# ChainBreak/denoising_diffusion_deep_fake

Measured on AMD Instinct MI355X. Metric: training images/sec (256x256 U-Net, bs=16/GPU), higher is better.
Workload: dtype f32; 1 GPU; d3f train_denoiser step: noise blend -> Unet(resnet34) fwd -> (MSE+1-SSIM)/2 -> bwd -> Adam, 256x256 synthetic face crops, bs=16/GPU, random-init weights, train-mode BatchNorm; image_size=256, batch_per_gpu=16, global_batch=16, parallelism=dp1, graph_step=False, adam_overlap_tail=False, adam_overlap_tail_steps=0, ranks_seen=1, csrc_digest=87bcf01c09701563

## Files before the change

### denoising_diffusion_deep_fake_amd/_lib.py

```python
import ctypes as C
import os
import re
from pathlib import Path

_HERE = Path(__file__).resolve().parent
LIB_PATH = Path(os.environ["D3F_LIB"]) if os.environ.get("D3F_LIB") else _HERE / "csrc" / "libd3f_hip.so"
HEADER_PATH = _HERE.parent / "include" / "d3f_hip.h"

F32, BF16, F32X3 = 0, 1, 2
AUGMENT_NONE = -1


ACT_IDENTITY, ACT_SIGMOID, ACT_TANH, ACT_SOFTMAX, ACT_LOGSOFTMAX, ACT_CLAMP = range(6)
HEAD_ACTIVATIONS = {None: ACT_IDENTITY, "sigmoid": ACT_SIGMOID, "tanh": ACT_TANH, "softmax2d": ACT_SOFTMAX,
                    "logsoftmax": ACT_LOGSOFTMAX, "clamp": ACT_CLAMP}


RESAMPLE_CUBIC, RESAMPLE_CUBIC_AA = 0, 1
COLOR_NONE, COLOR_MEANSTD = 0, 1
COLOR_MATCH_MODES = {None: COLOR_NONE, "none": COLOR_NONE, "meanstd": COLOR_MEANSTD}


def color_match_mode(color_match):
    if not (color_match is None or isinstance(color_match, str)) or color_match not in COLOR_MATCH_MODES:
# ... 129 lines not shown
    "d3f_paste_resize_cubic_u8": (_i, [_p, _i, _i, _i, _i64, _p, _i, _i, _i, _i, _i, _i, _i, _p, _p]),
    "d3f_channel_sums_u8": (_i, [_p, _i, _i, _i, _i64, _p, _p]),
    "d3f_color_match_coef": (_i, [_p, _p, _i, _i64, _p, _p]),
    "d3f_paste_resize_cubic_color_u8": (_i, [_p, _i, _i, _i, _i64, _p, _i, _i, _i, _i, _i, _i, _i, _p, _p, _p]),
    "d3f_temporal_filter_u8": (_i, [_p, _i64, _p, _i64, _i, _i, _i, _p, _p, _p, _f, _i, _p]),
    "d3f_color_coef_smooth": (_i, [_p, _p, _i, _i64, _f, _p, _p, _p, _p]),
    "d3f_temporal_flag_set": (_i, [_p, _i, _p]),
    "d3f_unet_predict_frames_full_u8": (_i, [_p, _p, _p, _p, _i, _i, _i, _i, _i, _i, _i, _p, _p, C.POINTER(_f), C.POINTER(_f),
                                             _p, _i, _p]),
    "d3f_crop_resize_cubic_boxes_u8": (_i, [_p, _i, _i, _i, C.POINTER(C.c_int32), _p, _i, _i, _i64, _p]),
    "d3f_crop_resize_cubic_aa_boxes_u8": (_i, [_p, _i, _i, _i, C.POINTER(C.c_int32), _p, _i, _i, _i64, _p]),
    "d3f_paste_resize_cubic_boxes_u8": (_i, [_p, _i, _i, _i, _i64, _p, _i, _i, C.POINTER(C.c_int32), _i, _p, _p]),
    "d3f_paste_resize_cubic_color_boxes_u8": (_i, [_p, _i, _i, _i, _i64, _p, _i, _i, C.POINTER(C.c_int32), _i, _p, _p, _p]),
    "d3f_unet_predict_frames_boxes_u8": (_i, [_p, _p, _p, _p, _i, _i, C.POINTER(C.c_int32), _p, C.POINTER(_f), C.POINTER(_f),
                                              _p, _i, _p]),
    "d3f_unet_predict_frames_full_boxes_u8": (_i, [_p, _p, _p, _p, _i, _i, C.POINTER(C.c_int32), _i, _p, _p, C.POINTER(_f),
                                                   C.POINTER(_f), _p, _i, _p]),
    "d3f_gray_decimate_u8": (_i, [_p, _i, _i, _i, _i, _p, _p]),
    "d3f_track_seed_u8": (_i, [_p, _i, _i, _i, _i, _i, _i, _i, _p, _p, _p]),
    "d3f_track_search_u8": (_i, [_p, _i, _i, _i, _i, _i, _i, _i, _i, _p, _p, _p, _p]),
    "d3f_track_template_u8": (_i, [_p, _i, _i, _i, _i, _i, _i, _i, _i, _i, _p, _p, _p, _p, _p]),
    "d3f_track_seed_scale_u8": (_i, [_p, _i, _i, _i, _i, _i, _i, _i, _p, _p, _p]),
    "d3f_track_search_scale_u8": (_i, [_p, _i, _i, _i, _i, _i, _i, _i, _i, _i, _i, _p, _p, _p, _p]),
    "d3f_track_template_scale_u8": (_i, [_p, _i, _i, _i, _i, _i, _i, _i, _i, _i, _i, _i, _p, _p, _p, _p, _p]),
    "d3f_image_grid_shape": (_i, [_i, _i, _i, _i, _i, C.POINTER(C.c_int32)]),
    "d3f_image_grid_u8": (_i, [C.POINTER(_p), _i, _i, _i, _i, _i, _i, _i, _i, _f, _f, _f, _p, _p]),
    "d3f_unet_num_segments": (_i, [_p]),
    "d3f_unet_plan_counts": (_i, [_p, C.POINTER(C.c_int32), C.POINTER(C.c_int32), C.POINTER(C.c_int32)]),
    "d3f_unet_segment_range": (_i, [_p, _i, C.POINTER(_i64), C.POINTER(_i64)]),
    "d3f_unet_backward": (_i, [_p, _p, _p, _p, _p, _i, _i, _p]),
    "d3f_unet_backward_nojoin": (_i, [_p, _p, _p, _p, _p, _i, _i, _p]),
    "d3f_unet_side_stream": (_i, [_p, C.POINTER(_p)]),
    "d3f_unet_backward_join": (_i, [_p, _p]),
    "d3f_adam_coefficients": (_i, [_f, _f, _f, _f, _i, _f, C.POINTER(_f)]),
    "d3f_unet_train_step": (_i, [_p, _p, _f, _f, _f, _p, _i, _p]),
    "d3f_unet_set_bn_sync": (_i, [_p, _p, _p, _i]),
    "d3f_unet_export": (_i, [_p, C.c_char_p, _p, _p, _p]),
    "d3f_unet_export_shape": (_i, [_p, C.c_char_p, C.POINTER(C.c_int32)]),
    "d3f_conv_upsample_folded": (_i, [_i, _p]),
    "d3f_conv_upsample_summed": (_i, [_i, _p]),
    "d3f_conv_packed_bytes": (_sz, [_i, _desc, _i]),
    "d3f_conv_pack_weights": (_i, [_i, _desc, _p, _p, _p, _p]),
    "d3f_conv_workspace_bytes": (_sz, [_i, _desc, _i]),
    "d3f_conv_stats_floats": (_sz, [_i, _desc, _i, C.POINTER(_i)]),
    "d3f_conv_forward": (_i, [_i, _desc, _p, _p, _p, _p, _p, _p, _p]),
    "d3f_conv_winograd_applies": (_i, [_i, _desc]),
    "d3f_conv_winograd_filter_bytes": (_sz, [_desc]),
    "d3f_conv_winograd_stats_floats": (_sz, [_desc, C.POINTER(_i)]),
    "d3f_conv_winograd_pack": (_i, [_desc, _p, _p, _p]),
    "d3f_conv_winograd_forward": (_i, [_desc, _p, _p, _p, _p, _p, _p, _p, _i, _p]),
    "d3f_conv_backward_data": (_i, [_i, _desc, _p, _p, _p, _p, _i, _i, _p, _p]),
    "d3f_conv_backward_weight_workspace_bytes": (_sz, [_i, _desc]),
    "d3f_conv_backward_weight": (_i, [_i, _desc, _p, _p, _p, _p, _p, _p]),
    "d3f_conv_layer_plan": (_i, [_i, _desc, _i, _cvp]),
    "d3f_unet_num_conv_layers": (_i, [_p]),
    "d3f_unet_conv_layer": (_i, [_p, _i, _desc, _cvp]),
    "d3f_bn_finalize": (_i, [_p, _i, _i, _i64, _p, _p, _p, _p, _p, _p]),
    "d3f_bn_apply": (_i, [_i, _p, _p, _i, _i64, _p, _i, _p, _p]),
    "d3f_bn_backward_workspace_bytes": (_sz, [_i, _i, _i64]),
    "d3f_bn_backward": (_i, [_i, _p, _p, _p, _p, _p, _i, _i64, _p, _p, _p, _p, _p, _p]),
    "d3f_bn_layer_plan": (_i, [_bnd, _bnp]),
    "d3f_bn_layer_forward": (_i, [_bnd, _p, _p, _p, _p, _p, _p, _p, _p, _p, _p, _p]),
    "d3f_bn_layer_backward": (_i, [_bnd, _p, _p, _p, _p, _p, _p, _p, _p, _i, _p, _p, _p]),
    "d3f_unet_bn_layer": (_i, [_p, _i, _bnd, _bnp]),
    "d3f_head_activation_forward": (_i, [_i, _p, _p, _i, _i, _i, _i, _p]),
    "d3f_head_activation_backward": (_i, [_i, _i, _p, _p, _p, _p, _i, _i, _i, _i, _i, _p]),
    "d3f_maxpool3x3s2_forward": (_i, [_i, _p, _p, _p, _i, _i, _i, _i, _p]),
    "d3f_maxpool3x3s2_backward": (_i, [_i, _p, _p, _p, _i, _i, _i, _i, _i, _p]),
    "d3f_upsample2x_backward": (_i, [_i, _p, _p, _i, _i, _i, _i, _p]),
    "d3f_nchw_to_nhwc": (_i, [_i, _p, _p, _i, _i, _i, _i, _i, _p]),
    "d3f_nhwc_to_nchw": (_i, [_i, _p, _p, _i, _i, _i, _i, _i, _p]),
    "d3f_noise_blend": (_i, [_p, _p, _p, _f, _p, _p, _i, _i64, _p]),
    "d3f_mse_ssim_loss_workspace_bytes": (_sz, [_i, _i, _i]),
    "d3f_mse_ssim_loss": (_i, [_p, _p, _f, _f, _p, _p, _p, _i, _i, _i, _p]),
    "d3f_adam_step": (_i, [_p, _p, _p, _p, _i64, _f, _f, _f, _f, _i, _f, _p]),
    "d3f_ema_lerp": (_i, [_p, _p, _i64, _f, _p]),
    "d3f_philox4x32_10": (_i, [_u32p, _u32p, _u32p]),
    "d3f_noise_blend_rng": (_i, [_p, _u64, _u64, _f, _p, _p, _i, _i64, _p]),
    "d3f_noise_blend_fixed_rng": (_i, [_p, _u64, _u64, _p, _p, _i, _i64, _p]),
    "d3f_noise_blend_fixed_index_rng": (_i, [_p, _u64, _u64, _p, _p, _p, _i, _i64, _p]),
    "d3f_noise_draw": (_i, [_u64, _u64, _p, _p, _i, _i64, _p]),
    "d3f_affine_warp_rng": (_i, [_p, _p, _u64, _u64, _i, C.POINTER(_f), _i, _i, _i, _i, _p]),
    "d3f_affine_theta_draw": (_i, [_u64, _u64, _i, C.POINTER(_f), _p, _p, _i, _i, _i, _p]),
    "d3f_pool_batch": (_i, [_p, _i64, _p, _p, _i, _i, _i, C.POINTER(_f), C.POINTER(_f), _p, _p, _p]),
    "d3f_pool_batch_rng": (_i, [_p, _i64, _p, _p, _i, _i, _i, C.POINTER(_f), C.POINTER(_f), _u64, _u64, _i, C.POINTER(_f), _p]),
    "d3f_pool_batch_balanced_rng": (_i, [_p, _i64, _p, _p, _i, _p, _p, _i, _i, _i, C.POINTER(_f), C.POINTER(_f), _u64, _u64, _i,
                                         C.POINTER(_f), _p]),
    "d3f_balanced_index_draw": (_i, [_p, _p, _i, _u64, _u64, _p, _i, _p]),
}

ALLREDUCE_FN = C.CFUNCTYPE(C.c_int, C.c_void_p, C.c_void_p, C.c_int64, C.c_void_p)

_lib = None


def header_symbols():
    text = HEADER_PATH.read_text()
    text = re.sub(r"/\*.*?\*/", "", text, flags=re.S)
    return sorted(set(re.findall(r"\b(d3f_[a-z0-9_]+)\s*\(", text)))


def sources_present():
    return HEADER_PATH.exists() and any((_HERE / "csrc").glob("*.hip"))


def source_digest():
# ... 58 lines not shown
```

### denoising_diffusion_deep_fake_amd/csrc/batchnorm.hip

```cpp
#include "common.h"
#include "pointwise.h"
#include "vec16.h"

#include <algorithm>
#include <type_traits>

namespace d3f {

constexpr float BN_EPS = 1e-5f, BN_MOMENTUM = 0.1f;

constexpr int BNF_SC = 32;
constexpr int BNF_MAX_ROWS = 1024;
#ifndef BNF_FWD_U_F32
#define BNF_FWD_U_F32 4
#endif
#ifndef BNF_BWD_U
#define BNF_BWD_U 2
#endif

__device__ __forceinline__ float2 bn_fwd_coef(double s1, double s2, double count, int c, const float* __restrict__ gamma,
                                              const float* __restrict__ beta, float eps, float momentum, bool store,
                                              float* __restrict__ running_mean, float* __restrict__ running_var,
                                              float* __restrict__ mean_o, float* __restrict__ invstd_o,
                                              float* __restrict__ scale_o, float* __restrict__ shift_o) {
// ... 636 lines not shown
      y4[u] = y4n[u];
      if (FROM_A) a4[u] = a4n[u];
      if (RD_DRES) d4[u] = d4n[u];
    }
  }
}

struct BnBwdOps {
  const float *mean, *invstd;
  float* k;
  const void* a;
  const float *mask_scale, *mask_shift;
};
static BnBwdOps bwd_ops(const BnLayer& L, const BnBufs& b) {
  const bool from_y = L.mask == BN_MASK_FROM_Y;
  return {bn_coef(b.coef, L.C, BN_MEAN), bn_coef(b.coef, L.C, BN_INVSTD), b.k != nullptr ? b.k : bn_coef(b.coef, L.C, BN_K),
          L.mask == BN_MASK_FROM_A ? b.a : nullptr, from_y ? bn_coef(b.coef, L.C, BN_SCALE) : nullptr,
          from_y ? bn_coef(b.coef, L.C, BN_SHIFT) : nullptr};
}

static int bn_bwd_finalize_apply_launch(const BnLayer& L, const BnBufs& b, const BnBwdOps& o, hipStream_t stream,
                                        const NetSplit* ns) {
  if (L.rows == 0) return 0;
  const NetSplit nv = net_split_or_single(ns);
  const dim3 grid((unsigned)((L.rows + L.rows_per_block - 1) / L.rows_per_block), (unsigned)(L.C / BNF_SC),
                  (unsigned)nv.nets);
  const bool from_a = o.mask_scale == nullptr && o.a != nullptr;
  const bool rd_dres = b.dres != nullptr && b.dres_acc;
  by_dtype(L.dtype, [&](auto* typed) {
    typedef std::remove_pointer_t<decltype(typed)> T;
    auto go = [&](auto kernel) {
      hipLaunchKernelGGL(kernel, grid, dim3(256), 0, stream, b.stats, L.bwd_rows, L.C, (double)L.rows, b.gamma, o.mean,
                         o.invstd, b.dgamma, b.dbeta, o.k, (const T*)b.dA, (const T*)o.a, (const T*)b.y, (T*)b.dy,
                         (T*)b.dres, L.rows, L.rows_per_block, o.mask_scale, o.mask_shift, nv);
    };
    if (from_a && rd_dres) go(bn_bwd_finalize_apply_kernel<T, true, true>);
    else if (from_a) go(bn_bwd_finalize_apply_kernel<T, true, false>);
    else if (rd_dres) go(bn_bwd_finalize_apply_kernel<T, false, true>);
    else go(bn_bwd_finalize_apply_kernel<T, false, false>);
  });
  D3F_HIP(hipGetLastError());
  return 0;
}

void bn_layer_plan(BnLayer& L) {
  static const bool no_fused = getenv("D3F_NO_BN_FUSED_FINALIZE") != nullptr;
  auto fused_ok = [&](int rows) {
    return L.allow_fused && !no_fused && (L.dtype == D3F_F32 || L.dtype == D3F_BF16) && L.C % BNF_SC == 0 && rows >= 1 &&
           rows <= BNF_MAX_ROWS;
  };
  const long min_rows = std::max(16L, 4L * (256 / std::max(1, std::min(256, L.C / (L.dtype == D3F_F32 ? 4 : 8)))));
  L.reduce_blocks = (int)std::clamp((L.rows + min_rows - 1) / min_rows, 1L, 1024L);
  L.bwd_rows = L.fused_rows > 0 ? L.fused_rows : L.reduce_blocks;
  L.fwd_fused = L.apply && fused_ok(L.fwd_rows);
  L.bwd_fused = fused_ok(L.bwd_rows);
  L.rows_per_block = L.fwd_fused || L.bwd_fused ? rows_per_block_for(L.rows, L.C / BNF_SC, L.dtype, L.plan_nets) : 0;
  L.stat_floats = (size_t)L.fwd_rows * L.Cpad * 2;
  L.part_floats = (size_t)std::max(L.reduce_blocks, L.fused_rows) * L.C * 2;
}

int bn_layer_finalize(const BnLayer& L, const BnBufs& b, long count, hipStream_t stream, const NetSplit* ns) {
  const NetSplit nv = net_split_or_single(ns);
  hipLaunchKernelGGL(bn_finalize_kernel, dim3(L.C, 1, nv.nets), dim3(256), 0, stream, b.stats, L.fwd_rows, L.C, L.Cpad,
                     (double)count, b.gamma, b.beta, BN_EPS, BN_MOMENTUM, b.running_mean, b.running_var,
                     bn_coef(b.coef, L.C, BN_MEAN), bn_coef(b.coef, L.C, BN_INVSTD), bn_coef(b.coef, L.C, BN_SCALE),
                     bn_coef(b.coef, L.C, BN_SHIFT), nv);
  D3F_HIP(hipGetLastError());
  return 0;
}

int bn_layer_apply(const BnLayer& L, const BnBufs& b, hipStream_t stream, const NetSplit* ns) {
  const int ve = L.dtype == D3F_F32 ? 4 : 8;
  D3F_CHECK(L.C % ve == 0 && (256 * ve) % L.C == 0, "bn_apply: C=%d must divide %d", L.C, 256 * ve);
  const long nvec = L.rows * L.C / ve;
  if (nvec == 0) return 0;
  const NetSplit nv = net_split_or_single(ns);
  const BnResidualOps r = residual_ops(L, b);
  by_dtype(L.dtype, [&](auto* typed) {
    typedef std::remove_pointer_t<decltype(typed)> T;
    auto go = [&](auto kernel) {
      hipLaunchKernelGGL(kernel, dim3(grid_for(nvec), 1, nv.nets), dim3(256), 0, stream, (const T*)b.y,
                         bn_coef(b.coef, L.C, BN_SCALE), bn_coef(b.coef, L.C, BN_SHIFT), (const T*)r.res, (const T*)r.yr,
                         r.scale_r, r.shift_r, L.relu ? 1 : 0, (T*)b.a, nvec, L.C, nv.ws);
    };
    if (r.res != nullptr) go(bn_apply_kernel<T, 1>);
    else if (r.yr != nullptr) go(bn_apply_kernel<T, 2>);
    else go(bn_apply_kernel<T, 0>);
  });
  D3F_HIP(hipGetLastError());
  return 0;
}

int bn_layer_forward(const BnLayer& L, const BnBufs& b, const BnSync* sync, hipStream_t stream, const NetSplit* ns) {
  long count = L.rows;
  if (sync != nullptr) {
    if (int rc = sync->fn(sync->ctx, b.stats, (int64_t)L.fwd_rows * L.Cpad * 2, (void*)stream))
      return set_error(rc, "BatchNorm statistics all-reduce failed in the forward pass (%s)", L.name.c_str());
    count *= sync->world;
  } else if (L.fwd_fused) {
    return bn_finalize_apply_launch(L, b, stream, ns);
  }
  if (int rc = bn_layer_finalize(L, b, count, stream, ns)) return rc;
  return L.apply ? bn_layer_apply(L, b, stream, ns) : 0;
}

int bn_layer_backward(const BnLayer& L, const BnBufs& b, const BnSync* sync, hipStream_t stream, const NetSplit* ns) {
  const int C = L.C, ve = L.dtype == D3F_F32 ? 4 : 8, vc = C / ve;
  const NetSplit nv = net_split_or_single(ns);
  const BnBwdOps o = bwd_ops(L, b);
  if (L.fused_rows == 0) {
    D3F_CHECK(C % ve == 0 && vc >= 1 && vc <= 256 && (256 % vc) == 0, "bn_bwd_reduce: unsupported channel count %d", C);
    by_dtype(L.dtype, [&](auto* typed) {
      typedef std::remove_pointer_t<decltype(typed)> T;
      hipLaunchKernelGGL(bn_bwd_reduce_kernel<T>, dim3(L.reduce_blocks, 1, nv.nets), dim3(256), 0, stream,
                         (const T*)b.dA, (const T*)o.a, (const T*)b.y, o.mean, o.invstd, b.stats, L.rows, C, o.mask_scale,
                         o.mask_shift, nv.ws);
    });
    D3F_HIP(hipGetLastError());
  }
  auto finalize = [&](long count, float* dgamma, float* dbeta) -> int {
    hipLaunchKernelGGL(bn_bwd_finalize_kernel, dim3(C, 1, nv.nets), dim3(256), 0, stream, b.stats, L.bwd_rows, C,
                       (double)count, b.gamma, o.invstd, dgamma, dbeta, o.k, nv);
    D3F_HIP(hipGetLastError());
    return 0;
  };
  if (sync != nullptr) {
    if (int rc = finalize(L.rows, b.dgamma, b.dbeta)) return rc;
    if (int rc = sync->fn(sync->ctx, b.stats, (int64_t)L.bwd_rows * C * 2, (void*)stream))
      return set_error(rc, "BatchNorm statistics all-reduce failed in the backward pass (%s)", L.name.c_str());
    if (int rc = finalize(L.rows * sync->world, nullptr, nullptr)) return rc;
  } else if (L.bwd_fused) {
    return bn_bwd_finalize_apply_launch(L, b, o, stream, ns);
  } else if (int rc = finalize(L.rows, b.dgamma, b.dbeta)) {
    return rc;
  }
  D3F_CHECK(C % ve == 0 && (256 * ve) % C == 0, "bn_bwd_apply: C=%d must divide %d", C, 256 * ve);
  const long nvec = L.rows * C / ve;
  if (nvec == 0) return 0;
  by_dtype(L.dtype, [&](auto* typed) {
    typedef std::remove_pointer_t<decltype(typed)> T;
    auto go = [&](auto kernel) {
      hipLaunchKernelGGL(kernel, dim3(grid_for(nvec), 1, nv.nets), dim3(256), 0, stream, (const T*)b.dA, (const T*)o.a,
                         (const T*)b.y, o.mean, o.invstd, o.k, (T*)b.dy, (T*)b.dres, nvec, C, o.mask_scale, o.mask_shift,
                         nv.ws);
    };
    const int mask = o.mask_scale != nullptr ? 1 : (o.a != nullptr ? 2 : 0);
    const int dres = b.dres == nullptr ? 0 : (b.dres_acc ? 2 : 1);
    auto by_dres = [&](auto m) {
      constexpr int M = decltype(m)::value;
      if (dres == 0) go(bn_bwd_apply_kernel<T, M, 0>);
      else if (dres == 1) go(bn_bwd_apply_kernel<T, M, 1>);
      else go(bn_bwd_apply_kernel<T, M, 2>);
    };
    if (mask == 0) by_dres(std::integral_constant<int, 0>());
    else if (mask == 1) by_dres(std::integral_constant<int, 1>());
    else by_dres(std::integral_constant<int, 2>());
// ... 7 lines not shown
```

### denoising_diffusion_deep_fake_amd/csrc/c_api.hip

```cpp
#include "../../include/d3f_hip.h"

#include <cstdarg>
#include <cstdio>
#include <cstring>
#include <new>
#include <vector>

#include "engine.h"
#include "head_act.h"
#include "philox.h"

namespace d3f {
static thread_local char g_err[1024] = "";
int set_error(int code, const char* fmt, ...) {
  va_list ap;
  va_start(ap, fmt);
  vsnprintf(g_err, sizeof(g_err), fmt, ap);
  va_end(ap);
  return code;
}
}

namespace d3f {
struct ProfRec {
// ... 464 lines not shown
  ConvLayer L;
  if (int rc = wino_plan(L, d)) return rc;
  D3F_CHECK(w && u && d->CinReal == d->C0, "conv_winograd_pack: null argument or padded input channels");
  return conv_winograd_pack_launch(w, reinterpret_cast<float*>(u), d->Cout, d->C0, (hipStream_t)stream);
}
int d3f_conv_winograd_forward(const d3f_conv_desc* d, const void* src0, const void* u, void* y, float* stats,
                              const float* scale, const float* shift, const void* residual, int relu, void* stream) {
  ConvLayer L;
  if (int rc = wino_plan(L, d)) return rc;
  if (d->B == 0) return 0;
  D3F_CHECK(src0 && u && y && ((scale == nullptr) == (shift == nullptr)), "conv_winograd_forward: null argument");
  D3F_CHECK(scale != nullptr || (residual == nullptr && relu == 0),
            "conv_winograd_forward: residual / ReLU belong to the eval epilogue (scale and shift)");
  ConvFwdBufs b;
  b.src0 = src0; b.w = u; b.out = y;
  if (scale != nullptr) {
    b.scale = scale; b.shift = shift; b.res = residual; b.relu = relu ? 1 : 0;
  } else {
    b.stats = stats;
  }
  return conv_layer_forward(L, b, true, (hipStream_t)stream);
}
int d3f_conv_backward_data(int dtype, const d3f_conv_desc* d, const void* dy, const void* w_dgrad,
                           void* dx0, void* dx1, int acc0, int acc1, void* workspace, void* stream) {
  ConvLayer L;
  const int sum2 = d != nullptr && d->upsample0 == 2 ? PLAN_SUM2 : 0;
  if (int rc = plan(L, dtype, d, PLAN_DGRAD | sum2 | (workspace ? PLAN_SPLITK : 0))) return rc;
  if (d->B == 0) return 0;
  D3F_CHECK(dy && w_dgrad && dx0 && (d->C1 == 0 || dx1), "conv_backward_data: null argument");
  ConvDgradBufs b;
  b.dy = dy; b.w = w_dgrad; b.dx0 = dx0; b.dx1 = dx1; b.acc0 = acc0; b.acc1 = acc1;
  b.w_skip = L.upfold ? reinterpret_cast<const char*>(w_dgrad) + L.wd4 : nullptr;
  b.slabs = reinterpret_cast<float*>(workspace);
  return conv_layer_dgrad(L, b, (hipStream_t)stream);
}
size_t d3f_conv_backward_weight_workspace_bytes(int dtype, const d3f_conv_desc* d) {
  ConvLayer L;
  return plan(L, dtype, d, PLAN_WGRAD) != 0 ? 0 : L.wslab_bytes;
}
int d3f_conv_backward_weight(int dtype, const d3f_conv_desc* d, const void* dy, const void* src0,
                             const void* src1, void* workspace, float* dw, void* stream) {
  ConvLayer L;
  if (int rc = plan(L, dtype, d, PLAN_WGRAD)) return rc;
  if (d->B == 0) {
    D3F_CHECK(dw, "conv_backward_weight: null argument");
    D3F_HIP(hipMemsetAsync(dw, 0, (size_t)d->Cout * d->CinReal * d->KH * d->KW * sizeof(float), (hipStream_t)stream));
    return 0;
  }
  D3F_CHECK(dy && src0 && workspace && dw && (d->C1 == 0 || src1), "conv_backward_weight: null argument");
  return wgrad_layer_launch(L.wl, dy, src0, src1, reinterpret_cast<float*>(workspace), dw, d->Cout, d->CinReal, dtype,
                            (hipStream_t)stream);
}

static void conv_launch_out(const ConvParams& p, int dtype, d3f_conv_launch_plan* o) {
  const bool igemm = p.patch == 0, smallc = igemm && conv_igemm_small_c(p, dtype);
  o->planned = 1;
  o->patch = p.patch; o->tile_bm = p.tile_bm; o->tile_bn = p.tile_bn; o->tiles_m = p.tiles_m; o->tiles_n = p.tiles_n;
  o->splitk = p.splitk; o->par = p.par; o->nz = p.nz;
  o->small_c = smallc ? 1 : 0;
  o->fast_addr = igemm && conv_igemm_fast_addr(p, smallc) ? 1 : 0;
  o->sum2 = p.sum2; o->stat_rows = p.stat_rows;
}
static void conv_layer_out(const ConvLayer& L, d3f_conv_plan* o) {
  o->upfold = L.upfold; o->parity = L.parity;
}
static void conv_fwd_out(const ConvLayer& L, d3f_conv_plan* o) {
  o->wino = L.wino; o->wino_rows = L.wino_rows;
  conv_launch_out(L.fwd, L.dtype, &o->fwd);
}
static void conv_dgrad_out(const ConvLayer& L, d3f_conv_plan* o) {
  if (L.upfold) conv_launch_out(L.dgrad_lo, L.dtype, &o->dgrad_lo);
  if (!L.upfold || L.C1 > 0) conv_launch_out(L.dgrad, L.dtype, &o->dgrad);
}
static void conv_wgrad_out(const ConvLayer& L, d3f_conv_plan* o) {
  o->wgrad_parts = L.wl.nparts;
  for (int i = 0; i < L.wl.nparts; ++i) {
    const WgradParams& w = L.wl.part[i];
    d3f_conv_wgrad_plan& q = o->wgrad[i];
    q.part = w.part; q.cls = w.cls; q.patch = w.patch; q.splits = w.splits; q.chunks_per_split = w.chunks_per_split;
    q.tile = wgrad_tile_edge(w); q.tiles = wgrad_tiles(w);
  }
}
int d3f_conv_layer_plan(int dtype, const d3f_conv_desc* d, int with_workspace, d3f_conv_plan* out) {
  D3F_CHECK(out != nullptr, "conv_layer_plan: null argument");
  std::memset(out, 0, sizeof(*out));
  ConvLayer G, F, D, W;
  if (int rc = plan(G, dtype, d, 0)) return rc;
  conv_layer_out(G, out);
  const int sk = with_workspace ? PLAN_SPLITK : 0;
  if (plan(F, dtype, d, PLAN_FWD | sk) == 0) conv_fwd_out(F, out);
  if (plan(D, dtype, d, PLAN_DGRAD | (d->upsample0 == 2 ? PLAN_SUM2 : 0) | sk) == 0) conv_dgrad_out(D, out);
  if (plan(W, dtype, d, PLAN_WGRAD) == 0) conv_wgrad_out(W, out);
  return 0;
}
int d3f_unet_num_conv_layers(d3f_unet_t h) { return h ? (int)h->e.units.size() : -1; }
int d3f_unet_conv_layer(d3f_unet_t h, int i, d3f_conv_desc* d, d3f_conv_plan* plan) {
  D3F_CHECK(h && d && plan && i >= 0 && i < (int)h->e.units.size(), "unet_conv_layer: index %d", i);
  const Unit& u = h->e.units[i];
  d->B = u.B; d->H = u.Hv; d->W = u.Wv; d->C0 = u.C0; d->C1 = u.C1;
  d->upsample0 = u.up0 ? (u.want_sum2 ? 2 : 1) : 0;
  d->Cout = u.Cout; d->KH = u.KH; d->KW = u.KW; d->stride = u.stride; d->pad = u.pad; d->CinReal = u.CinReal;
  std::memset(plan, 0, sizeof(*plan));
  conv_layer_out(u, plan);
  if (u.need_fwd) conv_fwd_out(u, plan);
  if (u.need_dgrad) conv_dgrad_out(u, plan);
  if (u.need_wgrad) conv_wgrad_out(u, plan);
// ... 527 lines not shown
```

### denoising_diffusion_deep_fake_amd/csrc/common.h

```cpp
#pragma once
#include <hip/hip_runtime.h>
#include <stdint.h>
#include <stddef.h>
#include <stdlib.h>

namespace d3f {

typedef uint16_t bf16_t;

typedef float f32x16 __attribute__((ext_vector_type(16)));
typedef float f32x4 __attribute__((ext_vector_type(4)));
typedef __bf16 bf16x8 __attribute__((ext_vector_type(8)));

}
#ifndef D3F_F32
#define D3F_F32 0
#define D3F_BF16 1
#define D3F_F32X3 2
#endif
namespace d3f {

static inline const char* prof_knob(const char* name) {
#ifdef D3F_PROFILING
  return getenv(name);
// ... 122 lines not shown
void prof_begin(int cls, double flops, hipStream_t s);
void prof_end(hipStream_t s);

enum ConvMode : int {
  CONV_RAW_STATS = 0,
  CONV_HEAD_NCHW = 1,
  CONV_EVAL_FUSED = 2,
  CONV_DGRAD = 3,
};

struct ConvParams {
  const void* src0;
  const void* src1;
  const void* w;
  void* out0;
  void* out1;
  float* stats;
  const float* scale;
  const float* shift;
  const void* res;
  unsigned src0_bytes, src1_bytes, w_bytes;
  int B, Hv, Wv;
  int C0, C1;
  int H0s, W0s;
  int shift0;
  int zi;
  int Ho, Wo, Cout;
  int CoutPad, Kpad;
  int w_ld;
  int par;
  int nz;
  int KH, KW, stride, pad;
  int M;
  int tiles_m, tiles_n;
  float* partial;
  int splitk;
  int stat_rows;
  int out_c0;
  int acc0, acc1;
  int mode;
  int relu;
  double flops;
  const void* bn_y;
  const float* bn_coef;
  float* bn_partial;
  const void* bn_a;
  unsigned div_howo_mul, div_howo_shr, div_wo_mul, div_wo_shr;
  int cin_real;
  int sum2;
  int patch;
  int nets, plan_nets;
  long net_ws, net_out0, net_scale;
  int tile_bm, tile_bn;
};
__device__ __forceinline__ ConvParams conv_params_of_net(const ConvParams& pin, int net) {
  ConvParams p = pin;
  if (net != 0) {
    net_shift(p.src0, p.net_ws); net_shift(p.src1, p.net_ws); net_shift(p.w, p.net_ws);
    net_shift(p.out0, p.net_out0); net_shift(p.out1, p.net_ws);
    net_shift(p.stats, p.net_ws); net_shift(p.scale, p.net_scale); net_shift(p.shift, p.net_ws);
    net_shift(p.res, p.net_ws); net_shift(p.partial, p.net_ws);
    net_shift(p.bn_y, p.net_ws); net_shift(p.bn_coef, p.net_ws); net_shift(p.bn_partial, p.net_ws); net_shift(p.bn_a, p.net_ws);
  }
  return p;
}

struct ConvTile {
  int BM, BN;
};
int conv_igemm_plan(ConvParams& p, int dtype, bool allow_splitk = false);
size_t conv_splitk_floats(const ConvParams& p);
int conv_igemm_launch(const ConvParams& p, int dtype, hipStream_t stream);
bool conv_igemm_small_c(const ConvParams& p, int dtype);
bool conv_igemm_fast_addr(const ConvParams& p, bool smallc);
bool conv_winograd_fits(const ConvParams& p, int dtype);
bool conv_winograd_applies(const ConvParams& p, int dtype);
int conv_winograd_stat_rows(const ConvParams& p);
size_t conv_winograd_filter_floats(const ConvParams& p);
int conv_winograd_pack_launch(const float* w , float* u, int Cout, int Cin, hipStream_t stream);
int conv_winograd_launch(const ConvParams& p , hipStream_t stream);
bool conv_pres_applies(const ConvParams& p, int dtype);
void conv_pres_plan(ConvParams& p);
int conv_pres_launch(const ConvParams& p, hipStream_t stream);
bool conv_patch_applies(const ConvParams& p, int dtype);
bool conv_stem_applies(const ConvParams& p, int dtype);
bool conv_stem_bf16_applies(const ConvParams& p, int dtype);
void conv_patch_plan(ConvParams& p, int dtype);
int conv_patch_launch(const ConvParams& p, hipStream_t stream);

struct WgradParams {
  const void* dy;
  const void* src0;
  const void* src1;
  float* partial;
  unsigned dy_bytes, src0_bytes, src1_bytes;
  int B, Hv, Wv, C0, C1, H0s, W0s, shift0;
  int Ho, Wo, Cout;
  int KH, KW, stride, pad;
  int M;
  int cin_real;
  int splits;
  int chunks_per_split;
  int tiles_co, tiles_ci;
  int patch;
  double flops;
  int part;
  int cls;
  int ci_base;
  int slab_cin;
  int slab_taps;
  int Mi, Hc, Wc;
  int step_img, step_row, step_col;
  int nets, plan_nets;
  long net_ws;
};
__device__ __forceinline__ WgradParams wgrad_params_of_net(const WgradParams& pin, int net) {
  WgradParams p = pin;
  if (net != 0) {
    net_shift(p.dy, p.net_ws); net_shift(p.src0, p.net_ws); net_shift(p.src1, p.net_ws); net_shift(p.partial, p.net_ws);
  }
  return p;
}
enum WgradPart : int { WG_WHOLE = 0, WG_CLASS = 1, WG_SKIP = 2 };
int wgrad_plan(WgradParams& p, int dtype);
size_t wgrad_partial_floats(const WgradParams& p);
int wgrad_tiles(const WgradParams& p);
int wgrad_tile_edge(const WgradParams& p);
int wgrad_launch(const WgradParams& p, int dtype, hipStream_t stream);

constexpr int WG_BATCH = 20;
struct WgradReduceJob {
  const float* partial;
  float* dw;
  int splits, CoutP, Cin, CinReal, taps, CB, nsg, VB, CinTot, c_off, fold, Cout, cz, block0, lds;
};
struct WgradReduceBatch {
  WgradReduceJob job[WG_BATCH];
  int n = 0, blocks = 0, lds = 0;
  int nets = 1;
  long net_ws = 0, net_grad = 0;
};
int wgrad_reduce_batch_add(WgradReduceBatch& tb, const float* partial, int splits, int CoutP, int Cout, int Cin,
                           int CinRealPart, int CinRealTotal, int c_off, int KH, int KW, int fold, float* dw);
int wgrad_reduce_batch_launch(const WgradReduceBatch& tb, hipStream_t stream);

struct WgradLayer {
  WgradParams part[2];
  int nparts;
};
int wgrad_layer_plan(WgradLayer& L, const WgradParams& base, int dtype);
size_t wgrad_layer_partial_floats(const WgradLayer& L);
int wgrad_layer_launch(const WgradLayer& L, const void* dy, const void* src0, const void* src1, float* partial,
                       float* dw, int CoutReal, int CinReal, int dtype, hipStream_t stream);
int wgrad_layer_launch_deferred(const WgradLayer& L, const void* dy, const void* src0, const void* src1, float* partial,
                                float* dw, int CoutReal, int CinReal, int dtype, WgradReduceBatch& tb,
                                hipStream_t stream, const NetSplit* ns = nullptr);

struct ConvLayer {
  int B = 0, Hv = 0, Wv = 0;
  int C0 = 0, C1 = 0, up0 = 0;
  int CinReal = 0, Cout = 0, KH = 0, KW = 0, stride = 1, pad = 0;
  int dtype = 0;
  bool head = false;
  bool need_fwd = false, need_dgrad = false, need_wgrad = false;
  bool want_sum2 = false;
  bool allow_splitk = false;
  int plan_nets = 0;
  int sdtype = 0;
  int Cin = 0, Ho = 0, Wo = 0, CoutPad = 0, Kpad = 0, CoutD = 0, KpadD = 0, CinRows = 0, C0Rows = 0, C1Rows = 0;
  bool upfold = false;
  bool parity = false;
  bool wino = false;
  ConvParams fwd{}, dgrad{}, dgrad_lo{};
  WgradLayer wl{};
  int wino_rows = 0;
  size_t wf = 0, wd = 0;
  size_t wfc = 0, wd4 = 0, wds = 0;
  size_t wu = 0;
  size_t splitk_floats = 0;
  size_t wslab_bytes = 0;
  double macs = 0;
};
int conv_layer_plan(ConvLayer& L);

struct ConvFwdBufs {
  const void* src0 = nullptr;
  const void* src1 = nullptr;
  const void* w = nullptr;
  void* out = nullptr;
  float* stats = nullptr;
  const float* bias = nullptr;
  const float* scale = nullptr;
  const float* shift = nullptr;
  const void* res = nullptr;
  int relu = 0;
  float* slabs = nullptr;
};
int conv_layer_forward(const ConvLayer& L, const ConvFwdBufs& b, bool wino, hipStream_t s, const NetSplit* ns = nullptr);
struct ConvDgradBufs {
  const void* dy = nullptr;
  const void* w = nullptr;
  const void* w_skip = nullptr;
  void* dx0 = nullptr;
  void* dx1 = nullptr;
  int acc0 = 0, acc1 = 0;
  float* slabs = nullptr;
  const void* bn_y = nullptr;
  const float* bn_coef = nullptr;
  float* bn_partial = nullptr;
  const void* bn_a = nullptr;
};
int conv_layer_dgrad(const ConvLayer& L, const ConvDgradBufs& b, hipStream_t s, const NetSplit* ns = nullptr);
struct PackEntry;
int conv_pack_entry(const ConvLayer& L, long w_off, size_t wf_off, size_t wd_off, bool fwd, bool dgrad, uint32_t block0,
                    PackEntry& e);

}
```

### denoising_diffusion_deep_fake_amd/csrc/conv_igemm.hip

```cpp
#include "common.h"

#include <cstdio>
#include <cstdlib>
#include <cstring>
#include <type_traits>
#include <utility>

namespace d3f {

template <typename T, int MT> struct Mma;
template <> struct Mma<float, 32> {
  using Acc = f32x16;
  static constexpr int NREG = 16;
  static constexpr int NINST = 4;
  template <typename F>
  static __device__ __forceinline__ void run(Acc& c, const uint4& a, const uint4& b, F&& after) {
    c = __builtin_amdgcn_mfma_f32_32x32x2f32(__uint_as_float(a.x), __uint_as_float(b.x), c, 0, 0, 0);
    after();
    c = __builtin_amdgcn_mfma_f32_32x32x2f32(__uint_as_float(a.y), __uint_as_float(b.y), c, 0, 0, 0);
    after();
    c = __builtin_amdgcn_mfma_f32_32x32x2f32(__uint_as_float(a.z), __uint_as_float(b.z), c, 0, 0, 0);
    after();
    c = __builtin_amdgcn_mfma_f32_32x32x2f32(__uint_as_float(a.w), __uint_as_float(b.w), c, 0, 0, 0);
    after();
// ... 1370 lines not shown
template <typename T, int BM, int BN, int WGM, int WGN, int MT, bool X3>
static int launch_cfg(const ConvParams& p, bool smallc, hipStream_t stream) {
  const dim3 grid((unsigned)(p.tiles_m * p.tiles_n), (unsigned)p.splitk, (unsigned)(p.nz * nets_of(p.nets))), block(256);
  const bool fast = conv_igemm_fast_addr(p, smallc);
  if (p.par == 3)
    hipLaunchKernelGGL((conv_igemm_kernel<T, BM, BN, WGM, WGN, MT, false, 2, X3>), grid, block, 0, stream, p);
  else if (smallc)
    hipLaunchKernelGGL((conv_igemm_kernel<T, BM, BN, WGM, WGN, MT, true, 0, X3>), grid, block, 0, stream, p);
  else if (fast)
    hipLaunchKernelGGL((conv_igemm_kernel<T, BM, BN, WGM, WGN, MT, false, 1, X3>), grid, block, 0, stream, p);
  else
    hipLaunchKernelGGL((conv_igemm_kernel<T, BM, BN, WGM, WGN, MT, false, 0, X3>), grid, block, 0, stream, p);
  D3F_HIP(hipGetLastError());
  return 0;
}

template <typename T, bool X3> static int launch_t(const ConvParams& p, bool smallc, hipStream_t stream) {
  const ConvTile t{p.tile_bm, p.tile_bn};
  D3F_CHECK(t.BM > 0 && t.BN > 0 && p.tiles_m == cdiv(p.M, t.BM) && p.tiles_n == cdiv(p.Cout, t.BN),
            "conv: params were not planned (tiles %d,%d)", p.tiles_m, p.tiles_n);
  if (t.BM == 256 && t.BN == 16) return launch_cfg<T, 256, 16, 4, 1, 16, X3>(p, smallc, stream);
  if (t.BM == 256 && t.BN == 32) return launch_cfg<T, 256, 32, 4, 1, 32, X3>(p, smallc, stream);
  if (t.BM == 128 && t.BN == 128) return launch_cfg<T, 128, 128, 2, 2, 32, X3>(p, smallc, stream);
  if (t.BM == 128 && t.BN == 64) return launch_cfg<T, 128, 64, 2, 2, 32, X3>(p, smallc, stream);
  if constexpr (!X3) {
    if (t.BM == 64 && t.BN == 32) return launch_cfg<T, 64, 32, 2, 1, 32, X3>(p, smallc, stream);
    if (t.BM == 32 && t.BN == 32) return launch_cfg<T, 32, 32, 1, 1, 32, X3>(p, smallc, stream);
  }
  D3F_CHECK(t.BM == 64 && t.BN == 64, "conv: no kernel for the %dx%d tile", t.BM, t.BN);
  return launch_cfg<T, 64, 64, 2, 2, 32, X3>(p, smallc, stream);
}

int conv_igemm_launch(const ConvParams& p, int dtype, hipStream_t stream) {
  if (p.M == 0) return 0;
  const bool smallc = is_small_c(p, dtype);
  ConvParams q = p;
  if (q.partial == nullptr) q.splitk = 1;
#ifdef D3F_PROFILING
  static const char* ablate = getenv("D3F_ABLATE_LOADS");
  if (ablate != nullptr) {
    if (ablate[0] == 'a' || ablate[0] == 'b') q.src0_bytes = q.src1_bytes = 0;
    if (ablate[0] == 'w' || ablate[0] == 'b') q.w_bytes = 0;
  }
#endif
  D3F_CHECK(q.nz >= 1 && (q.splitk == 1 || q.stat_rows == cdiv((long)q.nz * q.M, SK_ROWS)),
            "conv: split-K params were not planned");
  {
    unsigned m0, s0, m1, s1;
    fast_div_setup((unsigned)(q.Ho * q.Wo), &m0, &s0);
    fast_div_setup((unsigned)q.Wo, &m1, &s1);
    D3F_CHECK(m0 == q.div_howo_mul && s0 == q.div_howo_shr && m1 == q.div_wo_mul && s1 == q.div_wo_shr,
              "conv: output extent changed after the plan (%d x %d)", q.Ho, q.Wo);
  }
  const int prof_cls = q.mode == CONV_DGRAD ? PROF_CONV_DGRAD : PROF_CONV_FWD;
  const bool prof = prof_enabled(prof_cls);
  if (prof) prof_begin(prof_cls, q.flops, stream);
  int rc = q.patch >= 9       ? conv_pres_launch(q, stream)
           : q.patch          ? conv_patch_launch(q, stream)
           : dtype == D3F_F32X3 ? launch_t<float, true>(q, smallc, stream)
           : dtype == D3F_F32 ? launch_t<float, false>(q, smallc, stream)
                              : launch_t<bf16_t, false>(q, smallc, stream);
  if (prof) prof_end(stream);
  if (rc == 0 && q.splitk > 1) {
    const dim3 grid((unsigned)cdiv((long)q.nz * q.M, SK_ROWS), 1, (unsigned)nets_of(q.nets)), block(256);
    if (dtype != D3F_BF16)
      hipLaunchKernelGGL(conv_splitk_reduce_kernel<float>, grid, block, 0, stream, q);
    else
      hipLaunchKernelGGL(conv_splitk_reduce_kernel<bf16_t>, grid, block, 0, stream, q);
    if (hipGetLastError() != hipSuccess) rc = set_error(-2, "conv split-K reduce launch failed");
  }
  return rc;
}

}
```

### denoising_diffusion_deep_fake_amd/csrc/conv_patch.hip

```cpp
#include "common.h"

#include <cstdlib>

namespace d3f {

constexpr int CP_PH = 4, CP_PW = 64;

static bool patch_conv_off() {
  static const bool off = getenv("D3F_NO_PATCH_CONV") != nullptr;
  return off;
}

bool conv_patch_applies(const ConvParams& p, int dtype) {
  if (patch_conv_off() || (dtype != D3F_F32 && dtype != D3F_BF16)) return false;
  const bool mode_ok = p.mode == CONV_RAW_STATS || p.mode == CONV_HEAD_NCHW ||
                       (p.mode == CONV_EVAL_FUSED && p.res == nullptr) ||
                       (p.mode == CONV_DGRAD && p.out_c0 == p.Cout && (p.Cout % 4) == 0);
  const bool wide = p.C0 == 32 && dtype == D3F_BF16 && p.mode != CONV_HEAD_NCHW;
  const bool cin_ok = p.C0 == 16 || wide || (p.C0 == 4 && p.mode == CONV_DGRAD && dtype == D3F_F32) ||
                      (p.C0 == 8 && p.mode == CONV_DGRAD && dtype == D3F_BF16);
  const bool up = wide && p.shift0 == 1 && p.mode != CONV_DGRAD && p.Cout <= 16 && p.H0s * 2 == p.Hv && p.W0s * 2 == p.Wv;
  const bool sum2 = p.sum2 && dtype == D3F_BF16 && p.mode == CONV_DGRAD && p.C0 == 16 && p.Cout == 32 && p.shift0 == 0;
  if (p.sum2 && !sum2) return false;
  return mode_ok && p.par == 0 && p.KH == 3 && p.KW == 3 && p.stride == 1 && p.pad == 1 && cin_ok && p.C1 == 0 &&
         (p.shift0 == 0 || up) && p.zi == 0 && p.Cout <= (wide && !up ? 64 : sum2 ? 32 : 16) && (p.mode == CONV_HEAD_NCHW || (p.Cout % 4) == 0) &&
         p.Hv == p.Ho && p.Wv == p.Wo && (p.Ho % CP_PH) == 0 &&
         (p.Wo % CP_PW) == 0 && p.Kpad >= 9 * p.C0;
}

template <typename T, int CIN, int BN, bool UP = false, int CSRC = CIN, bool SUM2 = false>
__global__ __launch_bounds__(256) void conv_patch_kernel(const ConvParams pin) {
  const ConvParams p = conv_params_of_net(pin, (int)blockIdx.z);
  chain_priority();
  constexpr bool BF = sizeof(T) == 2;
  constexpr bool W64 = BF && CIN == 32;
  static_assert(!UP || (W64 && BN == 16), "up-sampled source: bf16 x 32 channels -> 16 filters");
  static_assert(CSRC == CIN || (BF && CIN == 16 && CSRC == 8 && !UP), "half-filled pixels: bf16, 8 of 16 channels");
  static_assert(!SUM2 || (BF && CIN == 16 && CSRC == 16 && BN == 32 && !UP), "2x2-summed data gradient: bf16 x 16 -> 32");
  static_assert(((CIN == 16 || (CIN == 4 && !BF)) && (BN == 16 || SUM2)) || (W64 && (BN == 32 || UP)),
                "16 channels (forward / data gradient of decoder block 4, head forward), fp32 x 4 (data gradient of the "
                "head) or bf16 x 32 -> 32 (decoder block 3 conv2)");
  constexpr int VEC = 16 / (int)sizeof(T);
  constexpr int PH = CP_PH, PW = CP_PW, PR = UP ? PH / 2 + 2 : PH + 2, PC = UP ? PW / 2 + 2 : PW + 2;
  constexpr int CS = W64 ? 20 : BF ? 10 : (CIN == 16 ? CIN + 4 : 12);
  constexpr int KR = 9 * CIN;
  constexpr int WS = W64 ? KR / 2 : BF ? KR / 2 + 2 : (CIN == 16 ? KR : KR + 4);
  constexpr int CV = CSRC / VEC;
  constexpr int KS = 9 * CSRC;
  constexpr int NPV = PR * PC * CV;
  constexpr int NWV = BN * (KS / VEC);
  constexpr int NLP = (NPV + 255) / 256, NLW = (NWV + 255) / 256;
  constexpr int BM = PH * PW, LDC = BN + 4, FM = PW / 16, NB = BN / 16;
  constexpr int PATCH_DW = PR * PC * CS > BM * LDC ? PR * PC * CS : BM * LDC;
  __shared__ __attribute__((aligned(16))) float lds[PATCH_DW + BN * WS];
  float* P = lds;
  float* Wl = lds + PATCH_DW;

  const int tid = threadIdx.x, lane = tid & 63, wave = tid >> 6;
  const int tiles_x = p.Wo / PW, tiles_y = p.Ho / PH;
  const int tile = (int)blockIdx.x;
  const int tx = tile % tiles_x, ty = (tile / tiles_x) % tiles_y, b = tile / (tiles_x * tiles_y);
  const int y0 = ty * PH, x0 = tx * PW;
  const int n0 = (int)blockIdx.y * BN;

  const __amdgpu_buffer_rsrc_t rs = make_rsrc(p.src0, p.src0_bytes);
  const __amdgpu_buffer_rsrc_t rw = make_rsrc(p.w, p.w_bytes);
  uint4 pv[NLP], wv[NLW];
#pragma unroll
  for (int i = 0; i < NLP; ++i) {
    const int id = tid + 256 * i;
    const int pix = id / CV, cv = id - pix * CV;
    const int pr = pix / PC, pc = pix - pr * PC;
    const int gy = (UP ? y0 / 2 : y0) - 1 + pr, gx = (UP ? x0 / 2 : x0) - 1 + pc;
    const int Hs = UP ? p.H0s : p.Hv, Ws = UP ? p.W0s : p.Wv;
    const bool ok = id < NPV && (unsigned)gy < (unsigned)Hs && (unsigned)gx < (unsigned)Ws;
    pv[i] = buf_load16(rs, ok ? (unsigned)(((b * Hs + gy) * Ws + gx) * CSRC + cv * VEC) * (unsigned)sizeof(T) : BUF_OOB);
  }
#pragma unroll
  for (int i = 0; i < NLW; ++i) {
    const int id = tid + 256 * i;
    const int row = id / (KS / VEC), ch = id - row * (KS / VEC);
    const bool ok = id < NWV && n0 + row < p.CoutPad;
    wv[i] = buf_load16(rw, ok ? (unsigned)((n0 + row) * p.w_ld + ch * VEC) * (unsigned)sizeof(T) : BUF_OOB);
  }
#pragma unroll
  for (int i = 0; i < NLP; ++i) {
    const int id = tid + 256 * i;
    const int pix = id / CV, cv = id - pix * CV;
    if (NPV % 256 == 0 || id < NPV) {
      if constexpr (BF && !W64) {
        *reinterpret_cast<uint2*>(&P[pix * CS + cv * 4]) = make_uint2(pv[i].x, pv[i].y);
        *reinterpret_cast<uint2*>(&P[pix * CS + cv * 4 + 2]) = make_uint2(pv[i].z, pv[i].w);
        if constexpr (CSRC < CIN) {
          *reinterpret_cast<uint2*>(&P[pix * CS + 4]) = make_uint2(0u, 0u);
          *reinterpret_cast<uint2*>(&P[pix * CS + 6]) = make_uint2(0u, 0u);
        }
      } else {
        *reinterpret_cast<uint4*>(&P[pix * CS + cv * 4]) = pv[i];
      }
    }
  }
#pragma unroll
  for (int i = 0; i < NLW; ++i) {
    const int id = tid + 256 * i;
    const int row = id / (KS / VEC), ch = id - row * (KS / VEC);
    if (NWV % 256 == 0 || id < NWV) {
      if constexpr (CSRC < CIN) {
        *reinterpret_cast<uint2*>(&Wl[row * WS + ch * 8]) = make_uint2(wv[i].x, wv[i].y);
        *reinterpret_cast<uint2*>(&Wl[row * WS + ch * 8 + 2]) = make_uint2(wv[i].z, wv[i].w);
        *reinterpret_cast<uint2*>(&Wl[row * WS + ch * 8 + 4]) = make_uint2(0u, 0u);
        *reinterpret_cast<uint2*>(&Wl[row * WS + ch * 8 + 6]) = make_uint2(0u, 0u);
      } else if constexpr (BF && !W64) {
        *reinterpret_cast<uint2*>(&Wl[row * WS + ch * 4]) = make_uint2(wv[i].x, wv[i].y);
        *reinterpret_cast<uint2*>(&Wl[row * WS + ch * 4 + 2]) = make_uint2(wv[i].z, wv[i].w);
      } else {
        const int chs = (CIN == 16 || W64) ? (ch ^ ((row >> 1) & 3)) : ch;
        *reinterpret_cast<uint4*>(&Wl[row * WS + chs * 4]) = wv[i];
      }
    }
  }
  __syncthreads();

  const int fr = lane & 15, fq = lane >> 4;
  f32x4 acc[FM * NB];
#pragma unroll
  for (int i = 0; i < FM * NB; ++i) acc[i] = f32x4{0.f, 0.f, 0.f, 0.f};
  if constexpr (UP) {
    const float* Bbase = Wl + fr * WS + (fq ^ ((fr >> 1) & 3)) * 4;
    const float* Acol[3];
#pragma unroll
    for (int kw = 0; kw < 3; ++kw) Acol[kw] = P + (((fr + kw - 1) >> 1) + 1) * CS + fq * 4;
#pragma unroll
    for (int tap = 0; tap < 9; ++tap) {
      const int kh = tap / 3, kw = tap - kh * 3;
      const int prow = ((wave + kh - 1) >> 1) + 1;
      const uint4 bb = *reinterpret_cast<const uint4*>(Bbase + tap * (CIN / 2));
      uint4 a[FM];
#pragma unroll
      for (int i = 0; i < FM; ++i) a[i] = *reinterpret_cast<const uint4*>(Acol[kw] + (prow * PC + 8 * i) * CS);
#pragma unroll
      for (int i = 0; i < FM; ++i)
        acc[i] = __builtin_amdgcn_mfma_f32_16x16x32_bf16(*reinterpret_cast<const bf16x8*>(&a[i]),
                                                         *reinterpret_cast<const bf16x8*>(&bb), acc[i], 0, 0, 0);
    }
  } else if constexpr (W64) {
    const float* Abase = P + (wave * PC + fr) * CS + fq * 4;
    const float* Bbase = Wl + fr * WS + (fq ^ ((fr >> 1) & 3)) * 4;
#pragma unroll
    for (int tap = 0; tap < 9; ++tap) {
// ... 573 lines not shown
        p.stats[((long)tile * p.CoutPad + n0 + tid) * 2 + 0] = a1;
        p.stats[((long)tile * p.CoutPad + n0 + tid) * 2 + 1] = a2;
      }
    }
  } else {
    const float4 sc = *reinterpret_cast<const float4*>(p.scale + n), sf = *reinterpret_cast<const float4*>(p.shift + n);
#pragma unroll
    for (int i = 0; i < NVEC; ++i) {
      const int row = rv0 + i * RSTEP;
      float4 v = *reinterpret_cast<const float4*>(&Cs[row * LDC + cv * 4]);
      v.x = v.x * sc.x + sf.x; v.y = v.y * sc.y + sf.y; v.z = v.z * sc.z + sf.z; v.w = v.w * sc.w + sf.w;
      if (p.relu) { v.x = fmaxf(v.x, 0.f); v.y = fmaxf(v.y, 0.f); v.z = fmaxf(v.z, 0.f); v.w = fmaxf(v.w, 0.f); }
      st4<bf16_t>(out + out_row(row) * p.Cout + n, v);
    }
  }
}

void conv_patch_plan(ConvParams& p, int dtype) {
  if (p.KH == 7) {
    p.patch = dtype == D3F_BF16 ? 8 : 2;
    p.nz = 1;
    p.splitk = 1;
    p.w_ld = p.Kpad;
    p.tiles_m = p.B * (p.Ho / ST_PH) * (p.Wo / ST_PW);
    p.tiles_n = p.Cout / ST_BN;
    p.stat_rows = p.tiles_m;
    return;
  }
  p.patch = dtype == D3F_BF16 ? (p.sum2 ? 7 : p.C0 == 32 ? (p.shift0 ? 5 : 4) : p.C0 == 8 ? 6 : 3) : 1;
  p.nz = 1;
  p.splitk = 1;
  p.w_ld = p.Kpad;
  p.tiles_m = p.B * (p.Ho / CP_PH) * (p.Wo / CP_PW);
  p.tiles_n = p.patch == 4 ? cdiv(p.Cout, 32) : 1;
  p.stat_rows = p.tiles_m;
}

int conv_patch_launch(const ConvParams& p, hipStream_t stream) {
  if (p.patch == 2 || p.patch == 8) {
    D3F_CHECK(p.tiles_m == p.B * (p.Ho / ST_PH) * (p.Wo / ST_PW) && p.tiles_n == p.Cout / ST_BN && p.C0 == (p.patch == 8 ? 8 : 4),
              "conv: stem patch params were not planned");
    const dim3 gs((unsigned)p.tiles_m, (unsigned)p.tiles_n, (unsigned)nets_of(p.nets));
    if (p.patch == 8) hipLaunchKernelGGL(conv_stem_bf16_kernel, gs, dim3(256), 0, stream, p);
    else hipLaunchKernelGGL(conv_stem_kernel, gs, dim3(256), 0, stream, p);
    D3F_HIP(hipGetLastError());
    return 0;
  }
  D3F_CHECK((p.patch == 1 || (p.patch >= 3 && p.patch <= 7)) && p.tiles_m == p.B * (p.Ho / CP_PH) * (p.Wo / CP_PW) &&
                (p.C0 == 16 || (p.C0 == 4 && p.patch == 1) || (p.C0 == 32 && (p.patch == 4 || p.patch == 5)) || (p.C0 == 8 && p.patch == 6)) &&
                p.Cout <= (p.patch == 4 ? 64 : p.patch == 7 ? 32 : 16) && (p.sum2 != 0) == (p.patch == 7) &&
                p.tiles_n == (p.patch == 4 ? cdiv(p.Cout, 32) : 1) &&
                (p.shift0 == 0) == (p.patch != 5),
            "conv: patch params were not planned");
  const dim3 g1((unsigned)p.tiles_m, 1, (unsigned)nets_of(p.nets)), g2((unsigned)p.tiles_m, (unsigned)p.tiles_n, (unsigned)nets_of(p.nets));
  if (p.patch == 7) hipLaunchKernelGGL((conv_patch_kernel<bf16_t, 16, 32, false, 16, true>), g1, dim3(256), 0, stream, p);
  else if (p.patch == 6) hipLaunchKernelGGL((conv_patch_kernel<bf16_t, 16, 16, false, 8>), g1, dim3(256), 0, stream, p);
  else if (p.patch == 5) hipLaunchKernelGGL((conv_patch_kernel<bf16_t, 32, 16, true>), g1, dim3(256), 0, stream, p);
  else if (p.patch == 4) hipLaunchKernelGGL((conv_patch_kernel<bf16_t, 32, 32>), g2, dim3(256), 0, stream, p);
  else if (p.patch == 3) hipLaunchKernelGGL((conv_patch_kernel<bf16_t, 16, 16>), g1, dim3(256), 0, stream, p);
  else if (p.C0 == 16) hipLaunchKernelGGL((conv_patch_kernel<float, 16, 16>), g1, dim3(256), 0, stream, p);
  else hipLaunchKernelGGL((conv_patch_kernel<float, 4, 16>), g1, dim3(256), 0, stream, p);
  D3F_HIP(hipGetLastError());
  return 0;
}

}
```

### denoising_diffusion_deep_fake_amd/csrc/conv_plan.hip

```cpp
#include "pointwise.h"

#include <algorithm>

namespace d3f {

int conv_layer_plan(ConvLayer& L) {
  D3F_CHECK(L.dtype == D3F_F32 || L.dtype == D3F_BF16 || L.dtype == D3F_F32X3, "conv: dtype %d", L.dtype);
  L.sdtype = L.dtype == D3F_F32X3 ? D3F_F32 : L.dtype;
  const int ve = L.sdtype == D3F_F32 ? 4 : 8, bke = L.sdtype == D3F_F32 ? 32 : 64;
  const size_t wsz = L.dtype == D3F_F32X3 ? 6 : L.sdtype == D3F_F32 ? 4 : 2;
  D3F_CHECK(L.B >= 0 && L.Hv > 0 && L.Wv > 0 && L.C0 > 0 && L.C1 >= 0 && L.Cout > 0, "conv: extent");
  D3F_CHECK(L.C0 % ve == 0 && L.C1 % ve == 0, "conv: channels must be multiples of %d", ve);
  D3F_CHECK(L.KH == L.KW && L.KH >= 1 && L.KH <= 7, "conv: kernel %dx%d", L.KH, L.KW);
  D3F_CHECK(L.stride == 1 || L.stride == 2, "conv: stride %d", L.stride);
  D3F_CHECK(!L.up0 || (L.Hv % 2 == 0 && L.Wv % 2 == 0), "conv: up-sampled extent must be even");
  D3F_CHECK(L.CinReal > 0 && L.CinReal <= L.C0 + L.C1, "conv: CinReal");

  const int B = L.B, K = L.KH;
  L.Cin = L.C0 + L.C1;
  L.Ho = (L.Hv + 2 * L.pad - K) / L.stride + 1;
  L.Wo = (L.Wv + 2 * L.pad - K) / L.stride + 1;
  L.CoutPad = (int)round_up(L.Cout, 16);
  L.Kpad = (int)round_up((long)K * K * L.Cin, bke);
  L.CoutD = (int)round_up(L.Cout, ve);
// ... 59 lines not shown
  D3F_CHECK(L.stride == 2 ? (L.Ho * 2 == L.Hv && L.Wo * 2 == L.Wv) : (L.Ho == L.Hv && L.Wo == L.Wv),
            "conv_backward_data: needs a 'same' (stride 1) or exactly halving (stride 2) conv");
  ConvParams dy{};
  dy.B = B; dy.C0 = L.CoutD;
  dy.mode = CONV_DGRAD;
  ConvParams& d = L.dgrad;
  if (L.upfold) {
    ConvParams& l = L.dgrad_lo;
    l = dy;
    l.Hv = l.H0s = L.Hv; l.Wv = l.W0s = L.Wv;
    l.Ho = L.Hv / 2; l.Wo = L.Wv / 2;
    l.Cout = l.out_c0 = L.C0; l.CoutPad = L.C0Rows; l.Kpad = 16 * L.CoutD;
    l.KH = l.KW = 4; l.stride = 2; l.pad = 1;
    l.M = B * l.Ho * l.Wo;
    if (int rc = plan(l, 2.0 * L.macs * L.C0 / L.Cin)) return rc;
    if (L.C1 == 0) return 0;
    d = dy;
    d.Hv = d.H0s = d.Ho = L.Hv; d.Wv = d.W0s = d.Wo = L.Wv;
    d.Cout = d.out_c0 = L.C1; d.CoutPad = L.C1Rows; d.Kpad = L.KpadD;
    d.KH = d.KW = 3; d.stride = 1; d.pad = 1;
    d.M = B * L.Hv * L.Wv;
    return plan(d, 2.0 * L.macs * L.C1 / L.Cin);
  }
  d = dy;
  d.Cout = L.Cin; d.CoutPad = L.CinRows; d.Kpad = L.KpadD;
  d.out_c0 = L.C1 > 0 ? L.C0 : L.Cin;
  if (L.parity) {
    d.par = K == 3 ? 1 : 2;
    d.Hv = d.Ho = d.H0s = L.Ho; d.Wv = d.Wo = d.W0s = L.Wo;
    d.KH = d.KW = K == 3 ? 2 : 1; d.stride = 1; d.pad = 0;
    d.M = B * L.Ho * L.Wo;
  } else {
    const int s2 = L.stride == 2 ? 1 : 0;
    d.Hv = L.Hv; d.Wv = L.Wv;
    d.H0s = L.Ho; d.W0s = L.Wo; d.shift0 = s2; d.zi = s2;
    d.Ho = L.Hv; d.Wo = L.Wv;
    d.KH = d.KW = K; d.stride = 1; d.pad = K - 1 - L.pad;
    d.M = B * L.Hv * L.Wv;
    d.sum2 = (L.want_sum2 && L.up0 && L.C1 == 0) ? 1 : 0;
  }
  return plan(d, 2.0 * L.macs);
}

static void net_conv(ConvParams& p, const NetSplit* ns) {
  if (ns != nullptr) {
    p.nets = ns->nets;
    p.net_ws = p.net_out0 = p.net_scale = ns->ws;
  }
}

int conv_layer_forward(const ConvLayer& L, const ConvFwdBufs& b, bool wino, hipStream_t s, const NetSplit* ns) {
  ConvParams p = L.fwd;
  p.src0 = b.src0; p.src1 = b.src1; p.w = b.w; p.out0 = b.out;
  net_conv(p, ns);
  if (L.head) {
    p.mode = CONV_HEAD_NCHW;
    p.scale = b.bias;
    if (ns != nullptr) {
      p.net_out0 = ns->out;
      p.net_scale = ns->par;
    }
    return conv_igemm_launch(p, L.dtype, s);
  }
  p.partial = p.splitk > 1 ? b.slabs : nullptr;
  if (b.scale != nullptr) {
    p.mode = CONV_EVAL_FUSED;
    p.scale = b.scale; p.shift = b.shift; p.res = b.res; p.relu = b.relu;
  } else {
    p.mode = CONV_RAW_STATS;
    p.stats = b.stats;
    if (wino) p.stat_rows = L.wino_rows;
  }
  return wino ? conv_winograd_launch(p, s) : conv_igemm_launch(p, L.dtype, s);
}

int conv_layer_dgrad(const ConvLayer& L, const ConvDgradBufs& b, hipStream_t s, const NetSplit* ns) {
  ConvParams p = L.upfold ? L.dgrad_lo : L.dgrad;
  p.src0 = b.dy; p.w = b.w; p.out0 = b.dx0; p.acc0 = b.acc0;
  if (!L.upfold) {
    p.out1 = b.dx1;
    p.acc1 = b.acc1;
  }
  p.partial = p.splitk > 1 ? b.slabs : nullptr;
  p.bn_y = b.bn_y; p.bn_coef = b.bn_coef; p.bn_partial = b.bn_partial; p.bn_a = b.bn_a;
  net_conv(p, ns);
  if (p.par == 2 && !p.acc0) {
    const NetSplit nv = net_split_or_single(ns);
    for (int n = 0; n < nv.nets; ++n)
      D3F_HIP(hipMemsetAsync(reinterpret_cast<char*>(b.dx0) + (size_t)n * nv.ws, 0,
                             (size_t)4 * p.M * p.Cout * (L.sdtype == D3F_F32 ? 4 : 2), s));
  }
  if (int rc = conv_igemm_launch(p, L.dtype, s)) return rc;
  if (!L.upfold || L.C1 == 0) return 0;
  ConvParams k = L.dgrad;
  k.src0 = b.dy; k.w = b.w_skip; k.out0 = b.dx1; k.acc0 = b.acc1;
  k.partial = k.splitk > 1 ? b.slabs : nullptr;
  net_conv(k, ns);
  return conv_igemm_launch(k, L.dtype, s);
}

int conv_pack_entry(const ConvLayer& L, long w_off, size_t wf_off, size_t wd_off, bool fwd, bool dgrad, uint32_t block0,
                    PackEntry& e) {
  const int taps = L.KH * L.KW;
  const long nf = fwd ? (long)L.CoutPad * L.Kpad : 0, nd = dgrad ? (long)L.CinRows * L.KpadD : 0;
  D3F_CHECK((!fwd || L.Kpad >= taps * L.Cin) && (!dgrad || L.KpadD >= taps * L.CoutD), "pack_weights: padded K too small");
  const int extent = std::max({L.Cout, L.CinReal, L.Cin, L.CoutPad, L.Kpad, L.CinRows, L.CoutD, L.KpadD});
// ... 34 lines not shown
```

### denoising_diffusion_deep_fake_amd/csrc/conv_wgrad.hip

```cpp
#include "common.h"

#include <cstdlib>
#include <cstring>

namespace d3f {

constexpr int KP = 32;

template <typename T> __device__ __forceinline__ void lds_store_as_f32(float* dst, const uint4& v);
template <> __device__ __forceinline__ void lds_store_as_f32<float>(float* dst, const uint4& v) {
  *reinterpret_cast<uint4*>(dst) = v;
}
template <> __device__ __forceinline__ void lds_store_as_f32<bf16_t>(float* dst, const uint4& v) {
  *reinterpret_cast<uint4*>(dst) = make_uint4(v.x << 16, v.x & 0xffff0000u, v.y << 16, v.y & 0xffff0000u);
  *reinterpret_cast<uint4*>(dst + 4) = make_uint4(v.z << 16, v.z & 0xffff0000u, v.w << 16, v.w & 0xffff0000u);
}

__device__ __forceinline__ void wg_split3x4(const uint4& v, uint2& h, uint2& m, uint2& l) {
  typedef float f32x2 __attribute__((ext_vector_type(2)));
  const uint32_t x[4] = {v.x, v.y, v.z, v.w};
  uint32_t r1[4], r2[4];
#pragma unroll
  for (int e = 0; e < 4; e += 2) {
    const f32x2 f = {__uint_as_float(x[e]), __uint_as_float(x[e + 1])};
// ... 460 lines not shown
  {
    const int hw = p.Hc * p.Wc, rem = KP % hw;
    p.step_img = KP / hw;
    p.step_row = rem / p.Wc;
    p.step_col = rem % p.Wc;
  }
  p.tiles_co = cdiv(p.Cout, t);
  p.tiles_ci = cdiv(p.slab_cin, t);
  const long base = (long)p.tiles_co * p.tiles_ci * p.slab_taps;
  const int total_chunks = wgrad_tiles(p);
  static const long target_env = prof_knob("D3F_WGRAD_TARGET") ? atol(prof_knob("D3F_WGRAD_TARGET")) : 0;
  const long target = (target_env > 0 ? target_env : (dtype == D3F_BF16 ? 1152 : 928)) / plan_nets_for(p.plan_nets, 16);
  long splits = (target + base - 1) / base;
  const long max_splits = (total_chunks + 3) / 4;
  if (splits > max_splits) splits = max_splits;
  if (splits < 1) splits = 1;
  p.chunks_per_split = cdiv(total_chunks, splits);
  p.splits = cdiv(total_chunks, p.chunks_per_split);
  return 0;
}

int wgrad_tiles(const WgradParams& p) { return p.patch ? wgrad_patch_tiles(p) : cdiv(p.Mi, KP); }
int wgrad_tile_edge(const WgradParams& p) { return p.patch ? 0 : pick_wtile(p); }

size_t wgrad_partial_floats(const WgradParams& p) {
  return (size_t)p.splits * p.Cout * p.slab_taps * p.slab_cin;
}

template <typename T>
static void wgrad_launch_t(const WgradParams& p, int bm, dim3 grid, hipStream_t stream, bool x3) {
  const dim3 block(256);
  if (bm == 64) {
    if (x3 || sizeof(T) == 2) {
      if (p.cls) hipLaunchKernelGGL((conv_wgrad_kernel<T, 64, 64, 2, 2, 1, true, true>), grid, block, 0, stream, p);
      else hipLaunchKernelGGL((conv_wgrad_kernel<T, 64, 64, 2, 2, 1, true>), grid, block, 0, stream, p);
      return;
    }
    if (p.cls) hipLaunchKernelGGL((conv_wgrad_kernel<T, 64, 64, 2, 2, 1, false, true>), grid, block, 0, stream, p);
    else hipLaunchKernelGGL((conv_wgrad_kernel<T, 64, 64, 2, 2, 1, false>), grid, block, 0, stream, p);
  } else {
    hipLaunchKernelGGL((conv_wgrad_kernel<T, 32, 32, 1, 1, 4, false>), grid, block, 0, stream, p);
  }
}

int wgrad_launch(const WgradParams& p, int dtype, hipStream_t stream) {
  if (p.M == 0) return 0;
  if (p.patch) {
    const bool prof = prof_enabled(PROF_WGRAD);
    if (prof) prof_begin(PROF_WGRAD, p.flops, stream);
    const int rc = wgrad_patch_launch(p, p.patch, dtype == D3F_F32X3 ? D3F_F32 : dtype, stream);
    if (prof) prof_end(stream);
    return rc;
  }
  const int t = pick_wtile(p);
  D3F_CHECK(p.tiles_co == cdiv(p.Cout, t) && p.splits >= 1 && p.slab_taps >= 1 && p.Mi >= 1, "wgrad: params were not planned");
  D3F_CHECK(!p.cls || t == 64, "wgrad: class form needs the 64x64 tile");
  const dim3 grid((unsigned)(p.tiles_ci * p.tiles_co * p.slab_taps), (unsigned)p.splits, (unsigned)nets_of(p.nets));
  const bool prof = prof_enabled(PROF_WGRAD);
  if (prof) prof_begin(PROF_WGRAD, p.flops, stream);
  if (dtype == D3F_BF16) wgrad_launch_t<bf16_t>(p, t, grid, stream, false);
  else wgrad_launch_t<float>(p, t, grid, stream, dtype == D3F_F32X3);
  if (prof) prof_end(stream);
  D3F_HIP(hipGetLastError());
  return 0;
}

static int wgrad_reduce_job(WgradReduceJob& q, const float* partial, int splits, int CoutP, int Cout, int Cin,
                            int CinRealPart, int CinRealTotal, int c_off, int KH, int KW, int fold, float* dw) {
  D3F_CHECK(Cin % 4 == 0 && CinRealPart <= Cin && Cout <= CoutP && c_off + CinRealPart <= CinRealTotal &&
                (!fold || (KH == 3 && KW == 3)),
            "wgrad reduce: arguments");
  const int taps = fold ? 16 : KH * KW;
  int cz = 1;
  while ((long)Cout * cz < 512 && Cin % (cz * 2) == 0 && Cin / (cz * 2) >= 16 && (Cin / (cz * 2)) % 4 == 0) cz *= 2;
  const int CB = Cin / cz, nvec = taps * CB / 4;
  int nsg = nvec >= 256 ? 1 : 256 / nvec;
  if (nsg > 8) nsg = 8;
  while (nsg > 1 && 2 * nsg > splits) --nsg;
  const int VB = nsg == 1 ? 256 : (nvec < 256 / nsg ? nvec : 256 / nsg);
  const size_t lds = (size_t)nsg * taps * (CB + 1) * sizeof(float);
  D3F_CHECK(lds <= 64 * 1024, "wgrad reduce: a %d-tap x %d-channel filter chunk exceeds the LDS tile", taps, CB);
  q.partial = partial; q.dw = dw;
  q.splits = splits; q.CoutP = CoutP; q.Cin = Cin; q.CinReal = CinRealPart; q.taps = taps; q.CB = CB; q.nsg = nsg;
  q.VB = VB; q.CinTot = CinRealTotal; q.c_off = c_off; q.fold = fold ? 1 : 0; q.Cout = Cout; q.cz = cz; q.block0 = 0;
  q.lds = (int)lds;
  return 0;
}

int wgrad_reduce_batch_add(WgradReduceBatch& tb, const float* partial, int splits, int CoutP, int Cout, int Cin,
                           int CinRealPart, int CinRealTotal, int c_off, int KH, int KW, int fold, float* dw) {
  D3F_CHECK(tb.n < WG_BATCH, "wgrad reduce batch: table full");
  WgradReduceJob& q = tb.job[tb.n];
  if (int rc = wgrad_reduce_job(q, partial, splits, CoutP, Cout, Cin, CinRealPart, CinRealTotal, c_off, KH, KW, fold, dw))
    return rc;
  q.block0 = tb.blocks;
  tb.blocks += q.Cout * q.cz;
  tb.lds = std::max(tb.lds, q.lds);
  ++tb.n;
  return 0;
}

int wgrad_reduce_batch_launch(const WgradReduceBatch& tb, hipStream_t stream) {
  if (tb.n == 0) return 0;
  hipLaunchKernelGGL(wgrad_reduce_batch_kernel, dim3((unsigned)tb.blocks, (unsigned)nets_of(tb.nets)), dim3(256), (size_t)tb.lds, stream, tb);
  D3F_HIP(hipGetLastError());
  return 0;
}

int wgrad_layer_plan(WgradLayer& L, const WgradParams& base, int dtype) {
  L.nparts = 1;
  L.part[0] = base;
  L.part[0].part = WG_WHOLE;
  if (wgrad_class_applies(base, dtype)) {
    L.part[0].part = WG_CLASS;
    L.part[0].flops = base.flops * base.C0 / (base.C0 + base.C1);
    if (base.C1 > 0) {
      L.nparts = 2;
      L.part[1] = base;
      L.part[1].part = WG_SKIP;
      L.part[1].flops = base.flops * base.C1 / (base.C0 + base.C1);
    }
  }
  for (int i = 0; i < L.nparts; ++i)
    if (int rc = wgrad_plan(L.part[i], dtype)) return rc;
  return 0;
}

size_t wgrad_layer_partial_floats(const WgradLayer& L) {
  size_t n = 0;
  for (int i = 0; i < L.nparts; ++i) n += (wgrad_partial_floats(L.part[i]) + 63) / 64 * 64;
  return n;
}

int wgrad_layer_launch_deferred(const WgradLayer& L, const void* dy, const void* src0, const void* src1, float* partial,
                                float* dw, int CoutReal, int CinReal, int dtype, WgradReduceBatch& tb,
                                hipStream_t stream, const NetSplit* ns) {
  if (ns != nullptr && ns->nets > 1) {
    tb.nets = ns->nets;
    tb.net_ws = ns->ws;
    tb.net_grad = ns->grad;
  }
  for (int i = 0; i < L.nparts; ++i) {
    WgradParams w = L.part[i];
    w.dy = dy; w.src0 = src0; w.src1 = src1; w.partial = partial;
    w.nets = ns != nullptr ? ns->nets : 1;
    w.net_ws = ns != nullptr ? ns->ws : 0;
    if (int rc = wgrad_launch(w, dtype, stream)) return rc;
    const int c_off = w.ci_base;
    const int creal = std::max(0, std::min(w.slab_cin, CinReal - c_off));
    if (int rc = wgrad_reduce_batch_add(tb, partial, w.splits, w.Cout, CoutReal, w.slab_cin, creal, CinReal, c_off, w.KH,
                                        w.KW, w.cls, dw))
      return rc;
    partial += (wgrad_partial_floats(w) + 63) / 64 * 64;
  }
  return 0;
}

int wgrad_layer_launch(const WgradLayer& L, const void* dy, const void* src0, const void* src1, float* partial,
                       float* dw, int CoutReal, int CinReal, int dtype, hipStream_t stream) {
  WgradReduceBatch tb;
  if (int rc = wgrad_layer_launch_deferred(L, dy, src0, src1, partial, dw, CoutReal, CinReal, dtype, tb, stream)) return rc;
  return wgrad_reduce_batch_launch(tb, stream);
}

}
```

### denoising_diffusion_deep_fake_amd/csrc/conv_wgrad_patch.hip

```cpp
#include "common.h"

#include <cstdlib>

namespace d3f {

constexpr int PT_TH = 8;

template <int MT> struct PAcc;
template <> struct PAcc<32> { using T = f32x16; static constexpr int N = 16; };
template <> struct PAcc<16> { using T = f32x4; static constexpr int N = 4; };

template <int MT> __device__ __forceinline__ void pmma(typename PAcc<MT>::T& c, float a, float b);
template <> __device__ __forceinline__ void pmma<32>(f32x16& c, float a, float b) {
  c = __builtin_amdgcn_mfma_f32_32x32x2f32(a, b, c, 0, 0, 0);
}
template <> __device__ __forceinline__ void pmma<16>(f32x4& c, float a, float b) {
  c = __builtin_amdgcn_mfma_f32_16x16x4f32(a, b, c, 0, 0, 0);
}

template <typename T> __device__ __forceinline__ void patch_store_f32(float* dst, const uint4& v);
template <> __device__ __forceinline__ void patch_store_f32<float>(float* dst, const uint4& v) {
  *reinterpret_cast<uint4*>(dst) = v;
}
template <> __device__ __forceinline__ void patch_store_f32<bf16_t>(float* dst, const uint4& v) {
  *reinterpret_cast<uint4*>(dst) = make_uint4(v.x << 16, v.x & 0xffff0000u, v.y << 16, v.y & 0xffff0000u);
  *reinterpret_cast<uint4*>(dst + 4) = make_uint4(v.z << 16, v.z & 0xffff0000u, v.w << 16, v.w & 0xffff0000u);
}

template <typename T, int MT, int CI_T, int KS, int S, int TW, int CR = CI_T>
__global__ __launch_bounds__(256) void conv_wgrad_patch_kernel(const WgradParams pin) {
  const WgradParams p = wgrad_params_of_net(pin, (int)blockIdx.z);
  constexpr int VE = Elem<T>::VE;
  constexpr int CO_T = MT;
  constexpr bool HALFV = CI_T < VE;
  static_assert(!HALFV || (CI_T == 4 && VE == 8), "half vectors: 4 of 8 bf16 channels");
  constexpr int PH = (PT_TH - 1) * S + KS, PW = (TW - 1) * S + KS;
  constexpr int KSTEP = (MT == 32) ? 2 : 4;
  static_assert(CR == CI_T || (CR < CI_T && CI_T < MT), "fewer columns than staged channels: small-channel path only");
  constexpr int NCOL = KS * KS * CR;
  constexpr int NNT = (NCOL + MT - 1) / MT;
  constexpr int LXS = (CI_T >= 32) ? (MT == 16 ? CI_T + 16 : CI_T + 4) : CI_T;
  constexpr int LYS = (MT == 32) ? CO_T + 4 : CO_T;
  constexpr int XF = PH * PW * LXS, YF = PT_TH * TW * LYS;
  constexpr int RED = 4 * MT * MT;
  constexpr int LDS_F = (XF + YF > RED) ? XF + YF : RED;
  __shared__ __attribute__((aligned(16))) float lds[LDS_F];
  float* Xs = lds;
  float* Ys = lds + XF;

  const int tid = threadIdx.x, lane = tid & 63, wave = tid >> 6;
  const int lc = lane & (MT - 1);
  const int lg = lane / MT;
  const int Cin = p.slab_cin;
  const int ci_slices = HALFV ? 1 : Cin / CI_T;
  const int slice = blockIdx.y;
  const int cil0 = (slice % ci_slices) * CI_T;
  const int ci0 = p.ci_base + cil0, co0 = (slice / ci_slices) * CO_T;
  const bool from0 = ci0 < p.C0;
  const int Cs = from0 ? p.C0 : p.C1;
  const int sh = from0 ? p.shift0 : 0;
  const int Hs = from0 ? p.H0s : p.Hv;
  const int Ws = from0 ? p.W0s : p.Wv;
  const int cl0 = from0 ? ci0 : ci0 - p.C0;
  const __amdgpu_buffer_rsrc_t rdy = make_rsrc(p.dy, p.dy_bytes);
  const __amdgpu_buffer_rsrc_t rx = from0 ? make_rsrc(p.src0, p.src0_bytes) : make_rsrc(p.src1, p.src1_bytes);

  int loff[(CI_T >= MT) ? 1 : NNT];
  if (CI_T < MT) {
#pragma unroll
    for (int j = 0; j < NNT; ++j) {
      const int n = j * MT + lc;
      int tap = n / CR;
      const int c = n - tap * CR;
      if (tap >= KS * KS) tap = KS * KS - 1;
      const int kh = tap / KS, kw = tap - kh * KS;
      loff[(CI_T >= MT) ? 0 : j] = (kh * PW + kw) * LXS + c;
    }
  }

  typename PAcc<MT>::T acc[NNT];
#pragma unroll
  for (int j = 0; j < NNT; ++j)
#pragma unroll
    for (int r = 0; r < PAcc<MT>::N; ++r) acc[j][r] = 0.f;

  const int tiles_x = (p.Wo + TW - 1) / TW, tiles_y = (p.Ho + PT_TH - 1) / PT_TH;
  const int ntiles = p.B * tiles_y * tiles_x;
  constexpr int VX = HALFV ? 1 : CI_T / VE, VY = CO_T / VE;

  constexpr int NVX = (PH * PW * VX + 255) / 256, NVY = (PT_TH * TW * VY + 255) / 256;
  uint4 rxv[NVX], ryv[NVY];
  auto issue_loads = [&](int t) {
    const int b = t / (tiles_y * tiles_x);
    const int tr = t - b * tiles_y * tiles_x;
    const int oy0 = (tr / tiles_x) * PT_TH, ox0 = (tr % tiles_x) * TW;
#pragma unroll
    for (int i = 0; i < NVX; ++i) {
      const int v = tid + i * 256;
      const int pix = v / VX, cv = v - pix * VX;
      const int py = pix / PW, px = pix - py * PW;
      const int iy = oy0 * S - p.pad + py, ix = ox0 * S - p.pad + px;
      const bool ok = v < PH * PW * VX && (unsigned)iy < (unsigned)p.Hv && (unsigned)ix < (unsigned)p.Wv;
      const int gp = (b * Hs + (iy >> sh)) * Ws + (ix >> sh);
      rxv[i] = buf_load16(rx, ok ? (unsigned)(gp * Cs + cl0 + cv * VE) * (unsigned)sizeof(T) : BUF_OOB);
    }
#pragma unroll
    for (int i = 0; i < NVY; ++i) {
      const int v = tid + i * 256;
      const int pix = v / VY, cv = v - pix * VY;
      const int y = pix / TW, x = pix - y * TW;
      const int oy = oy0 + y, ox = ox0 + x;
      const int co = co0 + cv * VE;
      const bool ok = v < PT_TH * TW * VY && oy < p.Ho && ox < p.Wo && co < p.Cout;
      ryv[i] = buf_load16(rdy, ok ? (unsigned)(((b * p.Ho + oy) * p.Wo + ox) * p.Cout + co) * (unsigned)sizeof(T) : BUF_OOB);
    }
  };
  auto store_tile = [&]() {
#pragma unroll
    for (int i = 0; i < NVX; ++i) {
      const int v = tid + i * 256;
      const int pix = v / VX, cv = v - pix * VX;
      if (v < PH * PW * VX) {
        if constexpr (HALFV)
          *reinterpret_cast<uint4*>(&Xs[pix * LXS]) =
              make_uint4(rxv[i].x << 16, rxv[i].x & 0xffff0000u, rxv[i].y << 16, rxv[i].y & 0xffff0000u);
        else
          patch_store_f32<T>(&Xs[pix * LXS + cv * VE], rxv[i]);
      }
    }
#pragma unroll
    for (int i = 0; i < NVY; ++i) {
      const int v = tid + i * 256;
      const int pix = v / VY, cv = v - pix * VY;
      if (v < PT_TH * TW * VY) patch_store_f32<T>(&Ys[pix * LYS + cv * VE], ryv[i]);
    }
  };

  if ((int)blockIdx.x < ntiles) issue_loads(blockIdx.x);
  for (int t = blockIdx.x; t < ntiles; t += gridDim.x) {
    __syncthreads();
    store_tile();
    __syncthreads();
    if (t + (int)gridDim.x < ntiles) issue_loads(t + gridDim.x);
#pragma unroll
    for (int yy = 0; yy < PT_TH / 4; ++yy) {
      const int y = wave * (PT_TH / 4) + yy;
      const float* __restrict__ yrow = Ys + (y * TW + lg) * LYS + lc;
      const float* __restrict__ xrow = Xs + ((y * S) * PW + lg * S) * LXS + ((CI_T >= MT) ? lc : 0);
#pragma unroll
      for (int xs = 0; xs < TW / KSTEP; ++xs) {
        const float a = yrow[xs * KSTEP * LYS];
        const float* __restrict__ xb = xrow + xs * KSTEP * S * LXS;
#pragma unroll
        for (int j = 0; j < NNT; ++j) {
          float bv;
          if (CI_T >= MT) {
            constexpr int per_tap = CI_T / MT;
            const int tap = j / per_tap, cb = (j % per_tap) * MT;
            const int kh = tap / KS, kw = tap % KS;
            bv = xb[(kh * PW + kw) * LXS + cb];
          } else {
            bv = xb[loff[(CI_T >= MT) ? 0 : j]];
          }
          pmma<MT>(acc[j], a, bv);
        }
      }
    }
  }

  const int taps = KS * KS;
  float* __restrict__ slab = p.partial + (long)blockIdx.x * p.Cout * taps * Cin;
  float* red = lds;
#pragma unroll
  for (int j = 0; j < NNT; ++j) {
    __syncthreads();
#pragma unroll
    for (int r = 0; r < PAcc<MT>::N; ++r) {
      const int co_l = (MT == 32) ? ((r & 3) + 8 * (r >> 2) + 4 * lg) : (4 * lg + r);
      red[(wave * MT + co_l) * MT + lc] = acc[j][r];
    }
// ... 266 lines not shown
    for (int r = 0; r < 16; ++r) red[(wave * 32 + (r & 3) + 8 * (r >> 2) + 4 * lh) * 32 + lc] = acc[j][r];
    __syncthreads();
    for (int e = tid; e < 32 * 32; e += 256) {
      const float sum = (red[e] + red[1024 + e]) + (red[2048 + e] + red[3072 + e]);
      const int co = co0 + (e >> 5), cil = e & 31;
      if (co < p.Cout && cil < xreal) slab[((long)co * taps + j) * Cin + cil0 + cil] = sum;
    }
  }
}

int wgrad_patch_variant(const WgradParams& p, int dtype) {
  const int cin = p.C0 + p.C1;
  if (p.KH != p.KW) return 0;
  constexpr int maxco = 128;
  constexpr int maxci = 384;
  if (dtype == D3F_BF16 && p.KH == 3 && p.stride == 1 && p.pad == 1 && p.Cout <= maxco && (cin == 16 || (cin % 32 == 0 && cin <= maxci)) &&
      (p.C1 == 0 || p.C0 % 32 == 0) && (p.C0 % 8) == 0 && (p.C1 % 8) == 0 && (p.Cout % 8) == 0)
    return 7;
  if (p.KH == 3 && p.stride == 1 && p.pad == 1) {
    if (p.Cout <= 16 && cin % 32 == 0 && cin <= 64 && (p.C1 == 0 || p.C0 % 32 == 0)) return 1;
    if (p.Cout <= 16 && cin == 16) return 2;
    if (p.Cout == 32 && cin % 32 == 0 && cin <= 128 && (p.C1 == 0 || p.C0 % 32 == 0)) return 3;
  }
  if (dtype == D3F_F32 && p.KH == 7 && p.stride == 2 && p.pad == 3 && cin == 4 && p.C1 == 0 &&
      p.Cout % 32 == 0 && p.Cout <= 64)
    return 4;
  if (dtype == D3F_BF16 && p.KH == 7 && p.stride == 2 && p.pad == 3 && cin == 8 && p.C1 == 0 &&
      p.Cout % 32 == 0 && p.Cout <= 64)
    return (p.cin_real > 0 && p.cin_real <= 4) ? 6 : 5;
  return 0;
}

int wgrad_patch_tiles(const WgradParams& p) { return p.B * cdiv(p.Ho, PT_TH) * cdiv(p.Wo, 16); }

void wgrad_patch_grid(const WgradParams& p, int variant, int* gx, int* gy) {
  const int cin = p.part == WG_WHOLE ? p.C0 + p.C1 : p.part == WG_CLASS ? p.C0 : p.C1;
  const int ci_t = variant == 1 ? 32 : variant == 2 ? 16 : (variant == 3 || variant == 7) ? 32 : (variant == 5 || variant == 6) ? 8 : 4;
  const int co_t = (variant == 3 || variant == 4 || variant == 5 || variant == 6 || variant == 7) ? 32 : 16;
  const int slices = cdiv(cin, ci_t) * cdiv(p.Cout, co_t) * (p.part == WG_CLASS ? 2 : 1);
  const int tiles = wgrad_patch_tiles(p);
  constexpr int g7 = 256;
  static const int gall = prof_knob("D3F_WGRAD_PATCH_WGS") ? atoi(prof_knob("D3F_WGRAD_PATCH_WGS")) : 512;
  int g = (variant == 7 ? g7 : gall) / plan_nets_for(p.plan_nets, 32) / slices;
  if (g > tiles) g = tiles;
  if (g < 1) g = 1;
  *gx = g;
  *gy = slices;
}

template <typename T> static int patch_launch_t(const WgradParams& p, int variant, dim3 grid, hipStream_t stream) {
  const dim3 block(256);
  switch (variant) {
    case 1: hipLaunchKernelGGL((conv_wgrad_patch_kernel<T, 16, 32, 3, 1, 16>), grid, block, 0, stream, p); break;
    case 2: hipLaunchKernelGGL((conv_wgrad_patch_kernel<T, 16, 16, 3, 1, 16>), grid, block, 0, stream, p); break;
    case 3: hipLaunchKernelGGL((conv_wgrad_patch_kernel<T, 32, 32, 3, 1, 16>), grid, block, 0, stream, p); break;
    default: return set_error(-1, "wgrad patch: bad variant %d", variant);
  }
  return 0;
}

int wgrad_patch_launch(const WgradParams& p, int variant, int dtype, hipStream_t stream) {
  int gx, gy;
  wgrad_patch_grid(p, variant, &gx, &gy);
  D3F_CHECK(p.splits == gx, "wgrad patch: params were not planned (splits %d vs %d)", p.splits, gx);
  const dim3 grid((unsigned)gx, (unsigned)gy, (unsigned)nets_of(p.nets)), block(256);
  if (p.cls) {
    D3F_CHECK((variant == 1 || variant == 3) && p.slab_cin == p.C0 && (p.C0 % 32) == 0 && (p.Ho % 2) == 0 && (p.Wo % 2) == 0,
              "wgrad patch: class form needs variant 1 or 3 and whole 32-channel slices of source 0");
    if (dtype == D3F_F32) {
      if (variant == 1) hipLaunchKernelGGL((conv_wgrad_patch_cls_kernel<float, 16, 32, 16>), grid, block, 0, stream, p);
      else hipLaunchKernelGGL((conv_wgrad_patch_cls_kernel<float, 32, 32, 16>), grid, block, 0, stream, p);
    } else {
      if (variant == 1) hipLaunchKernelGGL((conv_wgrad_patch_cls_kernel<bf16_t, 16, 32, 16>), grid, block, 0, stream, p);
      else hipLaunchKernelGGL((conv_wgrad_patch_cls_kernel<bf16_t, 32, 32, 16>), grid, block, 0, stream, p);
    }
    D3F_HIP(hipGetLastError());
    return 0;
  }
  if (variant == 7) {
    D3F_CHECK(dtype == D3F_BF16 && p.part == WG_WHOLE, "wgrad patch: variant 7 is the native bf16 kernel of whole layers");
    hipLaunchKernelGGL(conv_wgrad_patch_bf16_kernel, grid, block, 0, stream, p);
  } else if (variant == 4) {
    D3F_CHECK(dtype == D3F_F32, "wgrad patch: stem variant 4 is the f32 one");
    if (p.cin_real == 3) hipLaunchKernelGGL((conv_wgrad_patch_kernel<float, 32, 4, 7, 2, 16, 3>), grid, block, 0, stream, p);
    else hipLaunchKernelGGL((conv_wgrad_patch_kernel<float, 32, 4, 7, 2, 16>), grid, block, 0, stream, p);
  } else if (variant == 5) {
    D3F_CHECK(dtype == D3F_BF16, "wgrad patch: stem variant 5 is the bf16 one");
    hipLaunchKernelGGL((conv_wgrad_patch_kernel<bf16_t, 32, 8, 7, 2, 16>), grid, block, 0, stream, p);
  } else if (variant == 6) {
    D3F_CHECK(dtype == D3F_BF16, "wgrad patch: stem variant 6 is a bf16 one");
    if (p.cin_real == 3) hipLaunchKernelGGL((conv_wgrad_patch_kernel<bf16_t, 32, 4, 7, 2, 16, 3>), grid, block, 0, stream, p);
    else hipLaunchKernelGGL((conv_wgrad_patch_kernel<bf16_t, 32, 4, 7, 2, 16>), grid, block, 0, stream, p);
  } else if (dtype == D3F_F32) {
    if (int rc = patch_launch_t<float>(p, variant, grid, stream)) return rc;
  } else {
    if (int rc = patch_launch_t<bf16_t>(p, variant, grid, stream)) return rc;
  }
  D3F_HIP(hipGetLastError());
  return 0;
}

}
```

### denoising_diffusion_deep_fake_amd/csrc/engine.h

```cpp
#pragma once
#include <string>
#include <vector>

#include "common.h"
#include "pointwise.h"

namespace d3f {

struct TensorD {
  size_t off = 0;
  int H = 0, W = 0, C = 0;
  long elems(int B) const { return (long)B * H * W * C; }
};

struct ParamInfo {
  std::string name;
  int shape[4];
  int ndim;
  long offset;
  long numel;
};

struct BnInfo {
  std::string prefix;
  int C;
  long rm_off, rv_off;
};

struct Unit : ConvLayer {
  std::string conv_name;
  int in0 = -1, in1 = -1, y = -1, a = -1;
  bool bn = true, bias = false;
  BnLayer norm;
  int res_tensor = -1, res_unit = -1;
  long w_off = -1, bias_off = -1, g_off = -1, b_off = -1, rm_off = -1, rv_off = -1;
  size_t wf_off = 0, wd_off = 0;
  size_t coef_off = 0;
  int segment = 0;
  size_t dy_off = 0;
  size_t wfc_off = 0, wd4_off = 0, wds_off = 0;
  size_t wu_off = 0;
  size_t wslab_off = 0;
};

enum BwdKind { BW_HEAD, BW_UNIT, BW_SUM2X2, BW_POOL };
struct BwdOp {
  BwdKind kind;
  int unit = -1;
  int dA = -1;
  int fuse_for_unit = -1;
  int fused_rows = 0;
  bool mask = true;
  int dres = -1;
  bool dres_acc = false;
  int dst0 = -1, dst1 = -1;
  bool acc0 = false, acc1 = false;
  bool dst0_is_full_scratch = false;
  int C = 0, Hl = 0, Wl = 0;
  int segment = 0;
};

struct NetIO {
  long params = 0, bnstats = 0, grads = 0, x = 0, out = 0, dout = 0;
};

class UnetEngine {
 public:
  ~UnetEngine();
  int build(const char* encoder, int in_channels, int classes, int B, int H, int W, int dtype, int nets = 1,
            int plan_nets = 1);

  int pack_weights(const float* params, void* ws, hipStream_t s, const NetIO* io = nullptr) const;
  int forward(const float* params, float* bnstats, const float* x, float* out, void* ws, int training,
              hipStream_t s, const NetIO* io = nullptr) const;
  int backward(const float* params, const float* dout, float* grads, void* ws, int seg_begin,
               int seg_end, hipStream_t s, int join = 1, const NetIO* io = nullptr) const;
  int backward_join(hipStream_t s) const;
  hipStream_t side_stream() const;
  int predict_u8(const float* params, float* bnstats, const uint8_t* bgr_in, uint8_t* bgr_out,
                 const float mean[3], const float stdv[3], void* ws, int use_graph, hipStream_t s) const;
  struct FrameCall {
    const uint8_t* raw_in;
    int src_h, src_w, x1, y1, cw, ch;
    uint8_t* pair_out;
    uint8_t* full_out;
    int feather;
    const int32_t* boxes;
  };
  int predict_frames(const FrameCall& c, const float* params, float* bnstats, const float mean[3], const float stdv[3],
                     void* ws, int use_graph, hipStream_t s) const;
  int forward_graph(const float* params, float* bnstats, const float* x, float* out, void* ws, hipStream_t s) const;
  struct StepArgs {
    float* params; float* bnstats; float* grads; float* exp_avg; float* exp_avg_sq;
    const float* image; const float* noise; const float* y_uniform;
    float* noisy; float* pred; float* gpred; float* loss_out; float* loss_ws;
    const float* adam_coef;
    float lam, lo, hi;
  };
  int train_step(const StepArgs& a, void* ws, int use_graph, hipStream_t s) const;
  typedef int (*AllReduceFn)(void* ctx, float* data, int64_t count, void* stream);
  bool bn_sync_installed() const { return bn_sync_.fn != nullptr; }
  void set_bn_sync(AllReduceFn fn, void* ctx, int world) { bn_sync_ = BnSync{fn, ctx, world > 0 ? world : 1}; }
  int set_head_activation(int act);
  int head_activation() const { return head_act_; }
  enum { FRAME_RESAMPLE_CUBIC = 0, FRAME_RESAMPLE_CUBIC_AA = 1 };
  int set_frame_resample(int mode);
  int frame_resample() const { return frame_.resample; }
  enum { FRAME_COLOR_NONE = 0, FRAME_COLOR_MEANSTD = 1 };
  int set_frame_color_match(int mode);
  int frame_color_match() const { return frame_.color; }
  int set_frame_temporal(float strength, int threshold);
  float frame_temporal_strength() const { return frame_.strength; }
  int frame_temporal_threshold() const { return frame_.threshold; }
  int frame_temporal_reset(hipStream_t s) const;
  int export_tensor(const char* name, const void* ws, float* out_nchw, hipStream_t s) const;
  int export_shape(const char* name, int32_t dims[3]) const;

  std::vector<ParamInfo> params;
  std::vector<BnInfo> bns;
  long param_floats = 0, bnstat_floats = 0;
  size_t workspace_bytes = 0;
  int num_segments = 4;
  long seg_grad_begin[8] = {0}, seg_grad_end[8] = {0};
  int B = 0, H = 0, W = 0, dtype = 0, in_channels = 3, classes = 3;
  int nets = 1, plan_nets = 1;
  size_t net_ws_stride = 0;
  int cdtype = 0;
  double fwd_flops = 0, bwd_flops = 0;
  std::vector<Unit> units;

 private:
  int esize() const { return dtype == D3F_F32 ? 4 : 2; }
  int wsize() const { return cdtype == D3F_F32X3 ? 6 : esize(); }
  int ve() const { return dtype == D3F_F32 ? 4 : 8; }
  const TensorD* find_export(const char* name) const;
  int new_tensor(int H_, int W_, int C_);
  int new_grad(int tensor_id);
  size_t alloc(size_t bytes);
  int add_unit(const std::string& conv_name, const std::string& bn_name, int in0, int in1, int up0,
               int Cout, int k, int stride, int pad, bool bn, bool bias, bool relu, bool apply,
               int segment);

  std::vector<TensorD> tensors;
  std::vector<TensorD> gtensors;
  std::vector<int> grad_of;
  std::vector<bool> grad_init;
  std::vector<BwdOp> bwd_ops;
  std::vector<int> fwd_order_;
  mutable hipStream_t side_ = nullptr;
  mutable std::vector<hipEvent_t> ev_dy_;
  mutable hipEvent_t ev_join_ = nullptr;
  mutable hipEvent_t ev_seg_ = nullptr;
  mutable bool side_dirty_ = false;
  int ensure_streams() const;
  mutable hipEvent_t ev_pack_in_ = nullptr, ev_pack_done_ = nullptr, ev_pack_mid_ = nullptr;
  mutable bool pack_pending_ = false, pack_mid_pending_ = false;
  int first_mid_unit_ = -1;
  int first_late_unit_ = -1;
  int forward_body(const float* params, float* bnstats, float* out, char* ws, int training, hipStream_t s,
                   const NetSplit* ns = nullptr, bool apply_act = true) const;
  int head_to_u8bgr(const char* ws, uint8_t* out, long out_row_stride, const float mean255[3], const float std255[3],
                    hipStream_t s) const;
  void drop_graphs() const;
  void drop_frame_graphs() const;
  bool make_split(const NetIO* io, long in_delta, NetSplit* ns) const;
  int predict_u8_launches(const float* params, float* bnstats, const uint8_t* bgr_in, uint8_t* bgr_out,
                          const float mean255[3], const float std255[3], char* ws, hipStream_t s) const;
  struct GraphKey {
    const void* ptr[6];
    float cst[6];
    int geo[10];
  };
  struct GraphSlot {
    hipGraphExec_t exec = nullptr;
    GraphKey key = {};
    void destroy();
  };
  template <typename F>
  int graph_replay(GraphSlot& slot, const GraphKey& key, hipStream_t s, F&& launches) const;
  int wait_for_packed_weights(hipStream_t s) const;
  mutable hipStream_t gstream_ = nullptr;
  mutable GraphSlot g_predict_, g_eval_, g_frames_, g_frames_full_;
  BnSync bn_sync_{nullptr, nullptr, 1};
  const BnSync* bn_sync() const { return bn_sync_.fn != nullptr ? &bn_sync_ : nullptr; }
  int train_step_launches(const StepArgs& a, void* ws, hipStream_t s) const;
  mutable hipGraphExec_t g_step_ = nullptr;
  mutable StepArgs g_step_key_{};
  mutable const void* g_step_ws_ = nullptr;
  mutable hipEvent_t ev_gin_ = nullptr, ev_gout_ = nullptr;
  int head_act_ = 0;
  template <typename T>
  struct DevBuf {
    T* p = nullptr;
    DevBuf() = default;
    DevBuf(const DevBuf&) = delete;
    DevBuf& operator=(const DevBuf&) = delete;
    ~DevBuf() { if (p) (void)hipFree(p); }
    hipError_t ensure(size_t bytes) { return p ? hipSuccess : hipMalloc(reinterpret_cast<void**>(&p), bytes); }
  };
  struct FrameOptions {
    int resample = FRAME_RESAMPLE_CUBIC;
    int color = FRAME_COLOR_NONE;
    float strength = 0.f;
    int threshold = 8;
    mutable bool reset_pending = false;
    DevBuf<uint64_t> color_slabs;
    DevBuf<float> color_coef;
    DevBuf<float> state_fake;
    DevBuf<uint8_t> state_real;
    DevBuf<float> state_coef;
    DevBuf<uint64_t> state_sum;
    DevBuf<int> valid;
  };
  FrameOptions frame_;
  long pair_fake_off() const { return 3L * W; }
  long pair_stride() const { return 2 * pair_fake_off(); }
  size_t head_nchw_off = 0;
  mutable bool head_z_live_ = false;
  size_t ws_top = 0;
  int t_x = -1, t_pool = -1, head = -1, conv1 = -1;
  size_t pool_idx_off = 0, stats_off = 0, bnpart_off = 0, dz_off = 0, dfull_off = 0,
         bsum_off = 0, splitk_off = 0;
  size_t stats_bytes = 0, bnpart_bytes = 0, dy_bytes = 0, dz_bytes = 0, dfull_bytes = 0, splitk_bytes = 0;
};

int channel_sum_nchw_launch(const float* x, int B, int C, long HW, float* partial, float* out,
                            hipStream_t stream, const NetSplit* ns = nullptr);

}
```

### denoising_diffusion_deep_fake_amd/csrc/engine.hip

```cpp
#include "engine.h"
#include <vector>

#include "head_act.h"

#include <cstdio>
#include <cstdlib>
#include <cstring>

namespace d3f {

constexpr int CS_PP = 16;
__global__ __launch_bounds__(256) void channel_sum_partial_kernel(const float* __restrict__ x, int C, long HW,
                                                                  float* __restrict__ partial, int nb, long net_in,
                                                                  long net_ws) {
  __shared__ float red[256];
  const int seg = blockIdx.x, c = blockIdx.y, b = (int)blockIdx.z % nb;
  if ((int)blockIdx.z >= nb) {
    net_shift(x, net_in); net_shift(partial, net_ws);
  }
  const float* __restrict__ plane = x + ((long)b * C + c) * HW;
  const long per = (HW + CS_PP - 1) / CS_PP, lo = (long)seg * per, hi = lo + per < HW ? lo + per : HW;
  float s = 0.f;
  if ((HW & 3) == 0 && (per & 3) == 0) {
    for (long i = lo + 4 * threadIdx.x; i < hi; i += 4 * 256) {
// ... 288 lines not shown
    if (b.ud >= 0) dres = -2;
    else dres = grad_dst(u2.res_tensor, &dres_acc);
    if (int rc = emit_unit(b.u2, grad_of[u2.a], true, dres, dres_acc)) return rc;
    if (int rc = emit_unit(b.u1, grad_of[units[b.u1].a], true, -1, false)) return rc;
    if (b.ud >= 0)
      if (int rc = emit_unit(b.ud, -2, false, -1, false)) return rc;
  }
  {
    BwdOp p;
    p.kind = BW_POOL; p.segment = 3;
    p.dA = grad_of[t_pool];
    D3F_CHECK(p.dA >= 0, "plan: pool output without gradient");
    p.dst0 = grad_dst(f1, &p.acc0);
    bwd_ops.push_back(p);
  }
  if (int rc = emit_unit(conv1, grad_of[f1], true, -1, false)) return rc;

  static const bool no_fused_reduce = getenv("D3F_NO_FUSED_BN_REDUCE") != nullptr;
  if (!no_fused_reduce) {
    auto writes = [&](const BwdOp& o, int gid) {
      if (o.kind == BW_UNIT || o.kind == BW_HEAD) {
        if (units[o.unit].need_dgrad && !o.dst0_is_full_scratch && o.dst0 == gid) return true;
        if (o.dst1 == gid) return true;
        if (o.kind == BW_UNIT && o.dres == gid) return true;
      }
      return (o.kind == BW_SUM2X2 || o.kind == BW_POOL) && o.dst0 == gid;
    };
    for (size_t j = 0; j + 1 < bwd_ops.size(); ++j) {
      BwdOp& pj = bwd_ops[j];
      if (!(pj.kind == BW_UNIT || pj.kind == BW_HEAD)) continue;
      const Unit& up = units[pj.unit];
      const ConvParams& pd = up.upfold ? up.dgrad_lo : up.dgrad;
      if (!up.need_dgrad || pd.par || pj.dst0_is_full_scratch || (pj.dst1 >= 0 && !up.upfold) || pj.dst0 < 0) continue;
      BwdOp& ck = bwd_ops[j + 1];
      if (ck.kind != BW_UNIT || ck.dA != pj.dst0) continue;
      bool last = true;
      for (size_t k = j + 1; k < bwd_ops.size(); ++k) last = last && !writes(bwd_ops[k], pj.dst0);
      const Unit& uc = units[ck.unit];
      if (!last || !(uc.bn && ck.mask)) continue;
      D3F_CHECK(pd.Cout == uc.Cout && pd.M == (pd.sum2 ? 4 : 1) * B * uc.Ho * uc.Wo && pd.out_c0 == pd.Cout,
                "plan: fused BatchNorm reduce shape mismatch (%s -> %s)", up.conv_name.c_str(), uc.conv_name.c_str());
      pj.fuse_for_unit = ck.unit;
      ck.fused_rows = pd.splitk > 1 ? pd.stat_rows : pd.tiles_m;
    }
  }

  for (const BwdOp& op : bwd_ops) {
    if (op.kind != BW_UNIT) continue;
    Unit& u = units[op.unit];
    u.norm.res = u.res_tensor >= 0 ? BN_RES_TENSOR : u.res_unit >= 0 ? BN_RES_LAYER : BN_RES_NONE;
    u.norm.mask = !op.mask ? BN_MASK_NONE : u.norm.res == BN_RES_NONE ? BN_MASK_FROM_Y : BN_MASK_FROM_A;
    u.norm.fused_rows = op.fused_rows;
  }
  for (Unit& u : units) {
    if (!u.bn) continue;
    bn_layer_plan(u.norm);
    stats_bytes = std::max(stats_bytes, u.norm.stat_floats * sizeof(float));
    bnpart_bytes = std::max(bnpart_bytes, u.norm.part_floats * sizeof(float));
  }

  stats_off = alloc(stats_bytes);
  bnpart_off = alloc(bnpart_bytes);
  dz_off = alloc(dz_bytes);
  dfull_off = alloc(dfull_bytes);
  bsum_off = alloc(channel_sum_partial_floats(B, classes) * sizeof(float));
  splitk_off = alloc(splitk_bytes);
  head_nchw_off = alloc((size_t)B * classes * H * W * sizeof(float));
  net_ws_stride = nets > 1 ? (size_t)round_up((long)ws_top, 4096) : 0;
  workspace_bytes = nets > 1 ? net_ws_stride * nets : ws_top;

  long layer3_start = -1, layer4_start = -1, dec_start = -1;
  for (const auto& p : params) {
    if (layer3_start < 0 && p.name.rfind("encoder.layer3.", 0) == 0) layer3_start = p.offset;
    if (layer4_start < 0 && p.name.rfind("encoder.layer4.", 0) == 0) layer4_start = p.offset;
    if (dec_start < 0 && p.name.rfind("decoder.", 0) == 0) dec_start = p.offset;
  }
  num_segments = 4;
  seg_grad_begin[0] = dec_start;     seg_grad_end[0] = param_floats;
  seg_grad_begin[1] = layer4_start;  seg_grad_end[1] = dec_start;
  seg_grad_begin[2] = layer3_start;  seg_grad_end[2] = layer4_start;
  seg_grad_begin[3] = 0;             seg_grad_end[3] = layer3_start;
  fwd_order_.clear();
  fwd_order_.push_back(conv1);
  fwd_order_.push_back(-1);
  for (const auto& b : enc_blocks) {
    fwd_order_.push_back(b.u1);
    if (b.ud >= 0) fwd_order_.push_back(b.ud);
    fwd_order_.push_back(b.u2);
  }
  for (const auto& d : dec_blocks) {
    fwd_order_.push_back(d.u1);
    fwd_order_.push_back(d.u2);
  }
  fwd_order_.push_back(head);
  return 0;
}

static int shared_side_stream(hipStream_t* out) {
  constexpr int MAXDEV = 64;
  static hipStream_t streams[MAXDEV] = {};
  int dev = 0;
  D3F_HIP(hipGetDevice(&dev));
  D3F_CHECK(dev >= 0 && dev < MAXDEV, "side stream: device index %d", dev);
  if (streams[dev] == nullptr) {
    int least = 0, greatest = 0;
    D3F_HIP(hipDeviceGetStreamPriorityRange(&least, &greatest));
// ... 63 lines not shown
      char* ws = ws_of(n);
      if (t.n > 0)
        if (int rc = pack_all_launch(cdtype, params_, ws, t, (int)blocks, ps)) return rc;
      for (int ui = 0; ui < (int)units.size(); ++ui) {
        const Unit& u = units[ui];
        if (!u.wino) continue;
        if (first_late_unit_ > 0 ? part_of(ui) != part : part != 0) continue;
        if (int rc = conv_winograd_pack_launch(params_ + u.w_off, reinterpret_cast<float*>(ws + u.wu_off), u.Cout, u.Cin, ps))
          return rc;
      }
    }
    if (part == 1 && async) {
      D3F_HIP(hipEventRecord(ev_pack_mid_, side_));
      pack_mid_pending_ = true;
    }
    if (part == 2 || (first_late_unit_ <= 0 && part == 0)) {
      for (int n = 0; n < nets; ++n) {
        const float* params_ = params_of(n);
        char* ws = ws_of(n);
        for (const Unit& u : units)
          if (u.upfold)
            if (int rc = pack_up_launch(cdtype, params_ + u.w_off, u.Cout, u.C0, u.C1, ws + u.wfc_off, u.CoutPad,
                                        u.need_dgrad ? ws + u.wd4_off : nullptr, u.C0Rows,
                                        (u.need_dgrad && u.C1 > 0) ? ws + u.wds_off : nullptr, u.C1Rows, ps))
              return rc;
      }
    }
    if (part == 2 && async) {
      D3F_HIP(hipEventRecord(ev_pack_done_, side_));
      pack_pending_ = true;
    }
  }
  return 0;
}

int UnetEngine::forward(const float* params_, float* bnstats, const float* x, float* out, void* ws_,
                        int training, hipStream_t s, const NetIO* io) const {
  char* ws = reinterpret_cast<char*>(ws_);
  D3F_CHECK(nets == 1 || (io != nullptr && training), "unet: the pair engine runs train-mode passes and needs the second "
            "network's offsets");
  NetSplit split{};
  const NetSplit* ns = make_split(io, io ? io->x : 0, &split) ? &split : nullptr;
  if (int rc = nchw_to_nhwc_launch(dtype, x, ws + tensors[t_x].off, B, in_channels, H, W, tensors[t_x].C, s, ns))
    return rc;
  return forward_body(params_, bnstats, out, ws, training, s, ns);
}

int UnetEngine::forward_body(const float* params_, float* bnstats, float* out, char* ws, int training,
                             hipStream_t s, const NetSplit* ns, bool apply_act) const {
  auto T = [&](int tid) { return ws + tensors[tid].off; };
  auto coef = [&](const Unit& u) { return reinterpret_cast<float*>(ws + u.coef_off); };
  D3F_CHECK(ns == nullptr || (training && bn_sync() == nullptr), "unet: the pair engine runs train-mode passes with "
            "per-GPU BatchNorm statistics");
  if (!training) {
    BnEvalTable t;
    t.n = 0;
    for (const Unit& u : units)
      if (u.bn) {
        D3F_CHECK(t.n < PACK_MAX_LAYERS && u.coef_off % 16 == 0, "eval coefficients: table overflow");
        BnEvalEntry& e = t.e[t.n++];
        e.g_off = (uint32_t)u.g_off; e.b_off = (uint32_t)u.b_off;
        e.rm_off = (uint32_t)u.rm_off; e.rv_off = (uint32_t)u.rv_off;
        e.coef_off16 = (uint32_t)(u.coef_off >> 4);
        e.C = u.Cout;
      }
    if (int rc = bn_eval_coeff_all_launch(params_, bnstats, ws, t, s)) return rc;
  }
  for (int ui : fwd_order_) {
    if (ui < 0) {
      const TensorD& f1 = tensors[units[conv1].a];
      if (int rc = maxpool3x3s2_fwd_launch(dtype, T(units[conv1].a), T(t_pool),
                                           reinterpret_cast<uint8_t*>(ws + pool_idx_off), B, f1.H, f1.W,
                                           f1.C, s, ns))
        return rc;
      continue;
    }
    const Unit& u = units[ui];
    if (pack_mid_pending_ && ui >= first_mid_unit_) {
      D3F_HIP(hipStreamWaitEvent(s, ev_pack_mid_, 0));
      pack_mid_pending_ = false;
    }
    if (pack_pending_ && ui >= first_late_unit_) {
      D3F_HIP(hipStreamWaitEvent(s, ev_pack_done_, 0));
      pack_pending_ = false;
    }
    ConvFwdBufs b;
    b.src0 = T(u.in0);
    b.src1 = u.in1 >= 0 ? T(u.in1) : nullptr;
    b.w = ws + (u.wino ? u.wu_off : u.upfold ? u.wfc_off : u.wf_off);
    b.slabs = reinterpret_cast<float*>(ws + splitk_off);
    if (!u.bn) {
      b.bias = params_ + u.bias_off;
      if (head_act_ == HEAD_ACT_IDENTITY || !apply_act) {
        b.out = out;
        if (int rc = conv_layer_forward(u, b, false, s, ns)) return rc;
        continue;
      }
      float* z = reinterpret_cast<float*>(ws + head_nchw_off);
      NetSplit zs{};
      if (ns) {
        zs = *ns;
        zs.out = zs.ws;
      }
      b.out = z;
      if (int rc = conv_layer_forward(u, b, false, s, ns ? &zs : nullptr)) return rc;
      if (int rc = head_act_forward_launch(head_act_, z, out, B, u.Cout, u.Ho, u.Wo, s, ns)) return rc;
      head_z_live_ = training != 0;
      continue;
    }
    const Unit* ds = u.res_unit >= 0 ? &units[u.res_unit] : nullptr;
    if (training) {
      b.out = T(u.y);
      b.stats = reinterpret_cast<float*>(ws + stats_off);
      if (int rc = conv_layer_forward(u, b, u.wino, s, ns)) return rc;
      BnBufs n;
      n.stats = b.stats;
      n.gamma = params_ + u.g_off; n.beta = params_ + u.b_off;
      n.running_mean = bnstats + u.rm_off; n.running_var = bnstats + u.rv_off;
      n.coef = coef(u);
      n.y = T(u.y); n.a = u.a >= 0 ? T(u.a) : nullptr;
      n.res = u.res_tensor >= 0 ? T(u.res_tensor) : (ds ? T(ds->y) : nullptr);
      n.res_coef = ds ? coef(*ds) : nullptr;
      if (int rc = bn_layer_forward(u.norm, n, bn_sync(), s, ns)) return rc;
    } else {
      b.scale = bn_coef(coef(u), u.Cout, BN_SCALE);
      b.shift = bn_coef(coef(u), u.Cout, BN_SHIFT);
      b.relu = u.norm.relu ? 1 : 0;
      if (u.norm.apply) {
        b.out = T(u.a);
        b.res = u.res_tensor >= 0 ? T(u.res_tensor) : (ds ? T(ds->y) : nullptr);
      } else {
        b.out = T(u.y);
      }
      if (int rc = conv_layer_forward(u, b, u.wino, s, ns)) return rc;
    }
  }
  return 0;
}

int UnetEngine::predict_u8_launches(const float* params_, float* bnstats, const uint8_t* bgr_in, uint8_t* bgr_out,
                                    const float mean255[3], const float std255[3], char* ws, hipStream_t s) const {
  if (int rc = u8bgr_to_nhwc_launch(dtype, bgr_in, ws + tensors[t_x].off, (long)B * H * W, tensors[t_x].C, mean255,
                                    std255, s))
// ... 212 lines not shown
  return graph_replay(full ? g_frames_full_ : g_frames_, key, s, launches);
}

int UnetEngine::forward_graph(const float* params_, float* bnstats, const float* x, float* out, void* ws_,
                              hipStream_t s) const {
  const GraphKey key = {{params_, bnstats, x, out, ws_}, {}, {}};
  return graph_replay(g_eval_, key, s, [&](hipStream_t gs) { return forward(params_, bnstats, x, out, ws_, 0, gs); });
}

int UnetEngine::train_step_launches(const StepArgs& a, void* ws_, hipStream_t s) const {
  const long per_image = (long)in_channels * H * W;
  if (int rc = pack_weights(a.params, ws_, s)) return rc;
  if (int rc = noise_blend_launch(a.image, a.noise, a.y_uniform, a.lam, a.noisy, nullptr, B, per_image, s)) return rc;
  if (int rc = forward(a.params, a.bnstats, a.noisy, a.pred, ws_, 1, s)) return rc;
  if (int rc = mse_ssim_loss_launch(a.pred, a.image, a.lo, a.hi, a.loss_out, a.gpred, a.loss_ws, B, H, W, s)) return rc;
  if (int rc = backward(a.params, a.gpred, a.grads, ws_, 0, num_segments, s, 1)) return rc;
  return adam_step_dev_launch(a.params, a.grads, a.exp_avg, a.exp_avg_sq, param_floats, a.adam_coef, s);
}

int UnetEngine::train_step(const StepArgs& a, void* ws_, int use_graph, hipStream_t s) const {
  D3F_CHECK(in_channels == 3 && classes == 3, "train_step: the (MSE + 1 - SSIM) / 2 objective is defined on 3-channel images");
  if (!use_graph) return train_step_launches(a, ws_, s);
  if (int rc = wait_for_packed_weights(s)) return rc;
  if (int rc = ensure_streams()) return rc;
  if (gstream_ == nullptr) {
    D3F_HIP(hipStreamCreateWithFlags(&gstream_, hipStreamNonBlocking));
    D3F_HIP(hipEventCreateWithFlags(&ev_gin_, hipEventDisableTiming));
    D3F_HIP(hipEventCreateWithFlags(&ev_gout_, hipEventDisableTiming));
  }
  const bool same = g_step_ != nullptr && g_step_ws_ == ws_ && memcmp(&a, &g_step_key_, sizeof(StepArgs)) == 0;
  if (!same) {
    if (g_step_) {
      (void)hipGraphExecDestroy(g_step_);
      g_step_ = nullptr;
    }
    hipGraph_t graph = nullptr;
    D3F_HIP(hipStreamBeginCapture(gstream_, hipStreamCaptureModeThreadLocal));
    const int rc = train_step_launches(a, ws_, gstream_);
    const hipError_t e = hipStreamEndCapture(gstream_, &graph);
    pack_pending_ = pack_mid_pending_ = false;
    side_dirty_ = false;
    if (rc != 0) {
      if (graph) (void)hipGraphDestroy(graph);
      return rc;
    }
    D3F_HIP(e);
    const hipError_t ei = hipGraphInstantiate(&g_step_, graph, nullptr, nullptr, 0);
    (void)hipGraphDestroy(graph);
    D3F_HIP(ei);
    g_step_key_ = a;
    g_step_ws_ = ws_;
  }
  D3F_HIP(hipGraphLaunch(g_step_, s));
  return 0;
}

int UnetEngine::wait_for_packed_weights(hipStream_t s) const {
  if (pack_mid_pending_) {
    D3F_HIP(hipStreamWaitEvent(s, ev_pack_mid_, 0));
    pack_mid_pending_ = false;
  }
  if (pack_pending_) {
    D3F_HIP(hipStreamWaitEvent(s, ev_pack_done_, 0));
    pack_pending_ = false;
  }
  return 0;
}

template <typename F>
int UnetEngine::graph_replay(GraphSlot& slot, const GraphKey& key, hipStream_t s, F&& launches) const {
  if (int rc = wait_for_packed_weights(s)) return rc;
  if (gstream_ == nullptr) {
    D3F_HIP(hipStreamCreateWithFlags(&gstream_, hipStreamNonBlocking));
    D3F_HIP(hipEventCreateWithFlags(&ev_gin_, hipEventDisableTiming));
    D3F_HIP(hipEventCreateWithFlags(&ev_gout_, hipEventDisableTiming));
  }
  static_assert(sizeof(GraphKey) == 6 * sizeof(void*) + 6 * sizeof(float) + 10 * sizeof(int), "GraphKey is compared bytewise");
  const bool same = slot.exec != nullptr && memcmp(&key, &slot.key, sizeof(GraphKey)) == 0;
  if (!same) {
    slot.destroy();
    hipGraph_t graph = nullptr;
    D3F_HIP(hipStreamBeginCapture(gstream_, hipStreamCaptureModeThreadLocal));
    const int rc = launches(gstream_);
    const hipError_t e = hipStreamEndCapture(gstream_, &graph);
    if (rc != 0) {
      if (graph) (void)hipGraphDestroy(graph);
      return rc;
    }
    D3F_HIP(e);
    const hipError_t ei = hipGraphInstantiate(&slot.exec, graph, nullptr, nullptr, 0);
    (void)hipGraphDestroy(graph);
    D3F_HIP(ei);
    slot.key = key;
  }
  D3F_HIP(hipEventRecord(ev_gin_, s));
  D3F_HIP(hipStreamWaitEvent(gstream_, ev_gin_, 0));
  D3F_HIP(hipGraphLaunch(slot.exec, gstream_));
  D3F_HIP(hipEventRecord(ev_gout_, gstream_));
  D3F_HIP(hipStreamWaitEvent(s, ev_gout_, 0));
  return 0;
}

UnetEngine::~UnetEngine() {
  drop_graphs();
  if (ev_gin_) (void)hipEventDestroy(ev_gin_);
  if (ev_gout_) (void)hipEventDestroy(ev_gout_);
  if (gstream_) (void)hipStreamDestroy(gstream_);
  for (hipEvent_t e : ev_dy_)
    if (e) (void)hipEventDestroy(e);
  if (ev_join_) (void)hipEventDestroy(ev_join_);
  if (ev_seg_) (void)hipEventDestroy(ev_seg_);
  if (ev_pack_in_) (void)hipEventDestroy(ev_pack_in_);
  if (ev_pack_done_) (void)hipEventDestroy(ev_pack_done_);
  if (ev_pack_mid_) (void)hipEventDestroy(ev_pack_mid_);
}

static bool serial_backward() {
  static const bool serial = getenv("D3F_SERIAL_BACKWARD") != nullptr;
  return serial;
}

hipStream_t UnetEngine::side_stream() const {
  if (serial_backward() || ensure_streams() != 0) return nullptr;
  return side_;
}

int UnetEngine::backward_join(hipStream_t s) const {
  if (side_ != nullptr && side_dirty_) {
    D3F_HIP(hipEventRecord(ev_join_, side_));
    D3F_HIP(hipStreamWaitEvent(s, ev_join_, 0));
    side_dirty_ = false;
  }
  return 0;
}

int UnetEngine::backward(const float* params_, const float* dout, float* grads, void* ws_,
                         int seg_begin, int seg_end, hipStream_t s, int join, const NetIO* io) const {
  char* ws = reinterpret_cast<char*>(ws_);
  D3F_CHECK(nets == 1 || (io != nullptr && bn_sync() == nullptr), "unet: the pair engine needs the second network's "
            "offsets and runs with per-GPU BatchNorm statistics");
  NetSplit split{};
  const NetSplit* ns = make_split(io, io ? io->dout : 0, &split) ? &split : nullptr;
  const bool head_act = head_act_ != HEAD_ACT_IDENTITY;
  const float* head_dz = head_act ? reinterpret_cast<const float*>(ws + head_nchw_off) : dout;
  NetSplit split_dz = split;
  split_dz.in = split_dz.ws;
  const NetSplit* ns_dz = (ns && head_act) ? &split_dz : ns;
  auto T = [&](int tid) { return ws + tensors[tid].off; };
  auto G = [&](int gid) { return gid == -2 ? ws + dz_off : ws + gtensors[gid].off; };
  auto coef = [&](const Unit& u) { return reinterpret_cast<float*>(ws + u.coef_off); };
  const bool serial = serial_backward();
#ifdef D3F_PROFILING
  static const char* abl = getenv("D3F_ABLATE_BACKWARD");
  const bool skip_w = abl && strchr(abl, 'w'), skip_d = abl && strchr(abl, 'd'), skip_b = abl && strchr(abl, 'b');
  const bool skip_r = abl && strchr(abl, 'r');
#else
  constexpr bool skip_w = false, skip_d = false, skip_b = false, skip_r = false;
#endif
  if (!serial)
    if (int rc = ensure_streams()) return rc;
  hipStream_t ws_stream = serial ? s : side_;
  size_t next_event = 0;
  bool side_used = false;
  constexpr int defer = 3;
  std::vector<int> pending;
  int pending_segment = -1;
  bool head_bias_pending = false;
  auto flush_pending = [&]() -> int {
    if (pending.empty()) return 0;
    if (!serial) {
      if (next_event == ev_dy_.size()) {
        hipEvent_t e = nullptr;
        D3F_HIP(hipEventCreateWithFlags(&e, hipEventDisableTiming));
        ev_dy_.push_back(e);
      }
      D3F_HIP(hipEventRecord(ev_dy_[next_event], s));
      D3F_HIP(hipStreamWaitEvent(side_, ev_dy_[next_event], 0));
      ++next_event;
      side_used = true;
    }
    if (head_bias_pending) {
      const Unit& uh = units[head];
      if (int rc = channel_sum_nchw_launch(head_dz, B, uh.Cout, (long)uh.Ho * uh.Wo, reinterpret_cast<float*>(ws + bsum_off),
                                           grads + uh.bias_off, ws_stream, ns_dz))
        return rc;
      head_bias_pending = false;
    }
    for (int ui : pending) {
      const Unit& u = units[ui];
      WgradReduceBatch red;
      if (int rc = wgrad_layer_launch_deferred(u.wl, ws + u.dy_off, T(u.in0), u.in1 >= 0 ? T(u.in1) : nullptr,
                                               reinterpret_cast<float*>(ws + u.wslab_off), grads + u.w_off, u.Cout,
                                               u.CinReal, cdtype, red, ws_stream, ns))
        return rc;
      if (!skip_r)
        if (int rc = wgrad_reduce_batch_launch(red, ws_stream)) return rc;
    }
    pending.clear();
    return 0;
  };
  for (const BwdOp& op : bwd_ops) {
    if (op.segment < seg_begin || op.segment >= seg_end) continue;
    if (op.segment != pending_segment) {
      if (int rc = flush_pending()) return rc;
      pending_segment = op.segment;
    }
    if (op.kind == BW_SUM2X2) {
      if (int rc = sum2x2_launch(dtype, ws + dfull_off, G(op.dst0), B, op.Hl, op.Wl, op.C, s, ns)) return rc;
      continue;
    }
    if (op.kind == BW_POOL) {
      const TensorD& f1 = tensors[units[conv1].a];
      if (int rc = maxpool3x3s2_bwd_launch(dtype, G(op.dA), reinterpret_cast<uint8_t*>(ws + pool_idx_off),
                                           G(op.dst0), op.acc0 ? 1 : 0, B, f1.H, f1.W, f1.C, s, ns))
        return rc;
      continue;
    }
    const Unit& u = units[op.unit];
    char* dy = ws + u.dy_off;
    if (op.kind == BW_HEAD) {
      if (head_act) {
        D3F_CHECK(head_z_live_, "unet backward: the head's pre-activation output of the last training forward is gone (an "
                  "earlier backward pass turned it into dz, or an inference pass overwrote it): one backward pass per "
                  "training forward with an activated head");
        float* z = reinterpret_cast<float*>(ws + head_nchw_off);
        if (int rc = head_act_backward_launch(head_act_, dtype, z, dout, z, dy, B, u.Cout, u.Ho, u.Wo, u.CoutD, s, ns))
          return rc;
        head_z_live_ = false;
      } else {
        if (int rc = nchw_to_nhwc_launch(dtype, dout, dy, B, u.Cout, u.Ho, u.Wo, u.CoutD, s, ns)) return rc;
      }
      if (skip_w) {
        if (int rc = channel_sum_nchw_launch(head_dz, B, u.Cout, (long)u.Ho * u.Wo,
                                             reinterpret_cast<float*>(ws + bsum_off), grads + u.bias_off, s, ns_dz))
          return rc;
      } else {
        head_bias_pending = true;
      }
    } else if (!skip_b) {
      BnBufs n;
      n.stats = reinterpret_cast<float*>(ws + bnpart_off);
      n.gamma = params_ + u.g_off;
      n.coef = coef(u);
      n.y = T(u.y); n.a = u.a >= 0 ? T(u.a) : nullptr;
      n.dA = G(op.dA); n.dy = dy;
      n.dres = op.dres == -1 ? nullptr : G(op.dres); n.dres_acc = op.dres_acc ? 1 : 0;
      n.dgamma = grads + u.g_off; n.dbeta = grads + u.b_off;
      if (int rc = bn_layer_backward(u.norm, n, bn_sync(), s, ns)) return rc;
    }
    if (!skip_w) {
      pending.push_back(op.unit);
      if ((int)pending.size() >= defer)
        if (int rc = flush_pending()) return rc;
    }
    if (u.need_dgrad && !skip_d) {
      ConvDgradBufs d;
      d.dy = dy;
      d.w = ws + (u.upfold ? u.wd4_off : u.wd_off);
      d.w_skip = ws + u.wds_off;
      if (op.dst0_is_full_scratch) {
        d.dx0 = ws + dfull_off;
      } else {
        d.dx0 = G(op.dst0);
        d.acc0 = op.acc0 ? 1 : 0;
      }
      d.dx1 = op.dst1 >= 0 ? G(op.dst1) : nullptr;
      d.acc1 = op.acc1 ? 1 : 0;
      d.slabs = reinterpret_cast<float*>(ws + splitk_off);
      if (op.fuse_for_unit >= 0) {
        const Unit& uc = units[op.fuse_for_unit];
        d.bn_y = T(uc.y);
        d.bn_coef = bn_coef(coef(uc), uc.Cout, BN_MEAN);
        d.bn_partial = reinterpret_cast<float*>(ws + bnpart_off);
        d.bn_a = uc.norm.mask == BN_MASK_FROM_A ? T(uc.a) : nullptr;
      }
      if (int rc = conv_layer_dgrad(u, d, s, ns)) return rc;
    }
  }
  if (int rc = flush_pending()) return rc;
  if (!serial && side_used) side_dirty_ = true;
  if (!serial && !join) {
    D3F_HIP(hipEventRecord(ev_seg_, s));
    D3F_HIP(hipStreamWaitEvent(side_, ev_seg_, 0));
    side_dirty_ = true;
  } else if (!serial) {
    if (int rc = backward_join(s)) return rc;
  }
  return 0;
}

const TensorD* UnetEngine::find_export(const char* name) const {
  const std::string n(name);
  const size_t colon = n.rfind(':');
  if (colon == std::string::npos) return nullptr;
  const std::string un = n.substr(0, colon), kind = n.substr(colon + 1);
  if (kind != "y" && kind != "a" && kind != "da") return nullptr;
  for (const Unit& u : units) {
    if (u.conv_name != un) continue;
    const int tid = kind == "y" ? u.y : u.a;
    if (tid < 0) return nullptr;
    if (kind == "da") return grad_of[tid] >= 0 ? &gtensors[grad_of[tid]] : nullptr;
    return &tensors[tid];
  }
  return nullptr;
}

int UnetEngine::export_tensor(const char* name, const void* ws_, float* out_nchw, hipStream_t s) const {
  const TensorD* t = find_export(name);
  D3F_CHECK(t != nullptr, "export: no tensor named '%s' (expected '<conv name>:y|a|da')", name);
  return nhwc_to_nchw_launch(dtype, reinterpret_cast<const char*>(ws_) + t->off, out_nchw, B, t->C, t->H, t->W, t->C, s);
}

int UnetEngine::export_shape(const char* name, int32_t dims[3]) const {
  const TensorD* t = find_export(name);
  D3F_CHECK(t != nullptr, "export: no tensor named '%s' (expected '<conv name>:y|a|da')", name);
  dims[0] = t->C; dims[1] = t->H; dims[2] = t->W;
  return 0;
}

}
```

### denoising_diffusion_deep_fake_amd/csrc/pointwise.h

```cpp
#pragma once
#include <string>

#include "common.h"
#include "philox.h"

namespace d3f {

constexpr int PACK_MAX_LAYERS = 64;

enum BnCoefRow { BN_MEAN, BN_INVSTD, BN_SCALE, BN_SHIFT, BN_K, BN_COEF_ROWS = BN_K + 3 };
inline float* bn_coef(float* block, int C, BnCoefRow row) { return block + (long)row * C; }
inline const float* bn_coef(const float* block, int C, BnCoefRow row) { return block + (long)row * C; }

struct BnEvalEntry {
  uint32_t g_off, b_off, rm_off, rv_off;
  uint32_t coef_off16;
  int32_t C;
};
struct BnEvalTable {
  int n;
  BnEvalEntry e[PACK_MAX_LAYERS];
};
int bn_eval_coeff_all_launch(const float* params, const float* bnstats, void* ws, const BnEvalTable& t,
                             hipStream_t stream);

enum BnResidual { BN_RES_NONE, BN_RES_TENSOR, BN_RES_LAYER };
enum BnMask { BN_MASK_NONE, BN_MASK_FROM_Y, BN_MASK_FROM_A };
struct BnLayer {
  std::string name;
  int C = 0, Cpad = 0;
  long rows = 0;
  int dtype = D3F_F32;
  int plan_nets = 1;
  bool apply = true, relu = true;
  BnResidual res = BN_RES_NONE;
  BnMask mask = BN_MASK_NONE;
  int fwd_rows = 0;
  int fused_rows = 0;
  bool allow_fused = false;
  bool fwd_fused = false, bwd_fused = false;
  int reduce_blocks = 0;
  int bwd_rows = 0;
  long rows_per_block = 0;
  size_t stat_floats = 0;
  size_t part_floats = 0;
};
void bn_layer_plan(BnLayer& L);
struct BnBufs {
  float* stats = nullptr;
  const float *gamma = nullptr, *beta = nullptr;
  float *running_mean = nullptr, *running_var = nullptr;
  float* coef = nullptr;
  float* k = nullptr;
  const void* y = nullptr;
  void* a = nullptr;
  const void* res = nullptr;
  const float* res_coef = nullptr;
  const void* dA = nullptr;
  void* dy = nullptr;
  void* dres = nullptr;
  int dres_acc = 0;
  float *dgamma = nullptr, *dbeta = nullptr;
};
struct BnSync {
  int (*fn)(void* ctx, float* data, int64_t count, void* stream);
  void* ctx;
  int world;
};
int bn_layer_forward(const BnLayer& L, const BnBufs& b, const BnSync* sync, hipStream_t stream,
                     const NetSplit* ns = nullptr);
int bn_layer_backward(const BnLayer& L, const BnBufs& b, const BnSync* sync, hipStream_t stream,
                      const NetSplit* ns = nullptr);
int bn_layer_finalize(const BnLayer& L, const BnBufs& b, long count, hipStream_t stream, const NetSplit* ns = nullptr);
int bn_layer_apply(const BnLayer& L, const BnBufs& b, hipStream_t stream, const NetSplit* ns = nullptr);

int maxpool3x3s2_fwd_launch(int dtype, const void* in, void* out, uint8_t* idx, int B, int H, int W,
                            int C, hipStream_t stream, const NetSplit* ns = nullptr);
int maxpool3x3s2_bwd_launch(int dtype, const void* dout, const uint8_t* idx, void* din, int accumulate,
                            int B, int H, int W, int C, hipStream_t stream, const NetSplit* ns = nullptr);
int sum2x2_launch(int dtype, const void* dfull, void* dlow, int B, int Hl, int Wl, int C,
                  hipStream_t stream, const NetSplit* ns = nullptr);
int nchw_to_nhwc_launch(int dtype, const float* in, void* out, int B, int C, int H, int W, int Cpad,
                        hipStream_t stream, const NetSplit* ns = nullptr);
int nhwc_to_nchw_launch(int dtype, const void* in, float* out, int B, int C, int H, int W, int Cpad,
                        hipStream_t stream);

int u8bgr_to_nhwc_launch(int dtype, const uint8_t* in, void* out, long npix, int Cpad, const float mean255[3],
                         const float std255[3], hipStream_t stream);
int nchw_to_u8bgr_launch(const float* in, uint8_t* out, int B, int H, int W, long out_row_stride, const float mean255[3],
                         const float std255[3], hipStream_t stream);

int crop_resize_cubic_check(int B, int src_h, int src_w, int x1, int y1, int cw, int ch, int H, int W, long dst_row_stride);
// ... 264 lines not shown
```

### include/d3f_hip.h

```cpp
#ifndef D3F_HIP_H
#define D3F_HIP_H
#include <stddef.h>
#include <stdint.h>

#ifdef __cplusplus
extern "C" {
#endif

#define D3F_F32 0
#define D3F_BF16 1
#define D3F_F32X3 2

int d3f_version(void);
const char* d3f_last_error(void);
const char* d3f_source_digest(void);

int d3f_profile_enable(int max_launches);
int d3f_profile_classes(int mask);
int d3f_profile_collect(double ms[3], int64_t launches[3], double flops[3]);

typedef struct d3f_unet* d3f_unet_t;

int d3f_unet_create(const char* encoder_name, int in_channels, int classes, int B, int H, int W,
                    int dtype, d3f_unet_t* out);
// ... 70 lines not shown
int d3f_unet_backward_nojoin(d3f_unet_t h, const float* params, const float* grad_out, float* grads,
                             void* workspace, int seg_begin, int seg_end, void* stream);
int d3f_unet_side_stream(d3f_unet_t h, void** stream_out);
int d3f_unet_backward_join(d3f_unet_t h, void* stream);
typedef struct d3f_step_buffers {
  float* params; float* bnstats; float* grads; float* exp_avg; float* exp_avg_sq;
  const float* image;
  const float* noise;
  const float* y_uniform;
  float* noisy;
  float* pred;
  float* grad_pred;
  float* loss_out;
  void* loss_workspace;
  const float* adam_coef;
} d3f_step_buffers;
int d3f_adam_coefficients(float lr, float beta1, float beta2, float eps, int step, float grad_scale, float coef[8]);
int d3f_unet_train_step(d3f_unet_t h, const d3f_step_buffers* buffers, float lambda, float input_min, float input_max,
                        void* workspace, int use_graph, void* stream);
typedef int (*d3f_allreduce_fn)(void* ctx, float* data, int64_t count, void* stream);
int d3f_unet_set_bn_sync(d3f_unet_t h, d3f_allreduce_fn fn, void* ctx, int world_size);
int d3f_unet_export(d3f_unet_t h, const char* name, const void* workspace, float* out_nchw, void* stream);
int d3f_unet_export_shape(d3f_unet_t h, const char* name, int32_t dims[3]);

typedef struct d3f_conv_desc {
  int32_t B, H, W;
  int32_t C0, C1;
  int32_t upsample0;
  int32_t Cout, KH, KW, stride, pad;
  int32_t CinReal;
} d3f_conv_desc;

size_t d3f_conv_packed_bytes(int dtype, const d3f_conv_desc* d, int which);
int d3f_conv_pack_weights(int dtype, const d3f_conv_desc* d, const float* w, void* w_fwd, void* w_dgrad,
                          void* stream);
size_t d3f_conv_workspace_bytes(int dtype, const d3f_conv_desc* d, int which);
size_t d3f_conv_stats_floats(int dtype, const d3f_conv_desc* d, int with_workspace, int* tiles);
int d3f_conv_forward(int dtype, const d3f_conv_desc* d, const void* src0, const void* src1,
                     const void* w_fwd, void* y, float* stats, void* workspace, void* stream);
int d3f_conv_winograd_applies(int dtype, const d3f_conv_desc* d);
size_t d3f_conv_winograd_filter_bytes(const d3f_conv_desc* d);
size_t d3f_conv_winograd_stats_floats(const d3f_conv_desc* d, int* tiles);
int d3f_conv_winograd_pack(const d3f_conv_desc* d, const float* w, void* u, void* stream);
int d3f_conv_winograd_forward(const d3f_conv_desc* d, const void* src0, const void* u, void* y, float* stats,
                              const float* scale, const float* shift, const void* residual, int relu, void* stream);
int d3f_conv_upsample_folded(int dtype, const d3f_conv_desc* d);
int d3f_conv_upsample_summed(int dtype, const d3f_conv_desc* d);
int d3f_conv_backward_data(int dtype, const d3f_conv_desc* d, const void* dy, const void* w_dgrad,
                           void* dx0, void* dx1, int acc0, int acc1, void* workspace, void* stream);
size_t d3f_conv_backward_weight_workspace_bytes(int dtype, const d3f_conv_desc* d);
int d3f_conv_backward_weight(int dtype, const d3f_conv_desc* d, const void* dy, const void* src0,
                             const void* src1, void* workspace, float* dw, void* stream);

typedef struct d3f_conv_launch_plan {
  int32_t planned;
  int32_t patch;
  int32_t tile_bm, tile_bn;
  int32_t tiles_m, tiles_n, splitk;
  int32_t par, nz;
  int32_t small_c;
  int32_t fast_addr;
  int32_t sum2;
  int32_t stat_rows;
} d3f_conv_launch_plan;
typedef struct d3f_conv_wgrad_plan {
  int32_t part, cls;
  int32_t patch;
  int32_t splits;
  int32_t chunks_per_split;
  int32_t tile;
  int32_t tiles;
} d3f_conv_wgrad_plan;
typedef struct d3f_conv_plan {
  int32_t upfold;
  int32_t parity;
  int32_t wino, wino_rows;
  d3f_conv_launch_plan fwd, dgrad, dgrad_lo;
  int32_t wgrad_parts;
  d3f_conv_wgrad_plan wgrad[2];
} d3f_conv_plan;
int d3f_conv_layer_plan(int dtype, const d3f_conv_desc* d, int with_workspace, d3f_conv_plan* out);
int d3f_unet_num_conv_layers(d3f_unet_t h);
int d3f_unet_conv_layer(d3f_unet_t h, int i, d3f_conv_desc* d, d3f_conv_plan* plan);

int d3f_bn_finalize(const float* stats, int tiles, int C, int64_t count, const float* gamma,
                    const float* beta, float* running_mean, float* running_var, float* coef, void* stream);
int d3f_bn_apply(int dtype, const void* y, const float* coef, int C, int64_t rows, const void* residual,
                 int relu, void* out, void* stream);
size_t d3f_bn_backward_workspace_bytes(int dtype, int C, int64_t rows);
int d3f_bn_backward(int dtype, const void* dA, const void* a_or_null, const void* y, const float* coef,
                    const float* gamma, int C, int64_t rows, void* dy, void* dres, float* dgamma,
                    float* dbeta, void* workspace, void* stream);

typedef struct d3f_bn_desc {
  int32_t dtype, C, Cpad;
  int64_t rows;
  int32_t apply, relu;
  int32_t res;
  int32_t mask;
  int32_t fwd_rows;
  int32_t fused_rows;
  int32_t allow_fused, plan_nets;
} d3f_bn_desc;
typedef struct d3f_bn_plan {
  int32_t fwd_fused, bwd_fused;
  int32_t reduce_blocks;
// ... 157 lines not shown
```

Baseline: 2085 images/sec.

## Apply BatchNorm+ReLU while staging source tiles in fp32 16-channel patch convs

When a train-mode BN+ReLU output feeds only fp32 16-channel patch-conv consumers, the normalized activation is no longer written. The consumer conv forward and weight-gradient kernels now read the raw pre-BN tensor and apply scale, shift and ReLU as they stage tiles into shared memory. This removes a full-resolution elementwise pass and its write and read of the activation. The cost is extra per-element math in the staging loops, and exports of that activation must now recompute it on demand.

```diff
diff --git a/denoising_diffusion_deep_fake_amd/_lib.py b/denoising_diffusion_deep_fake_amd/_lib.py
--- a/denoising_diffusion_deep_fake_amd/_lib.py
+++ b/denoising_diffusion_deep_fake_amd/_lib.py
@@ -205,6 +205,10 @@
     "d3f_conv_backward_data": (_i, [_i, _desc, _p, _p, _p, _p, _i, _i, _p, _p]),
     "d3f_conv_backward_weight_workspace_bytes": (_sz, [_i, _desc]),
     "d3f_conv_backward_weight": (_i, [_i, _desc, _p, _p, _p, _p, _p, _p]),
+    "d3f_conv_source_bn_applies": (_i, [_i, _desc, _i]),
+    "d3f_conv_forward_source_bn": (_i, [_i, _desc, _p, _p, _p, _p, _p, _p, _p]),
+    "d3f_conv_backward_weight_source_bn": (_i, [_i, _desc, _p, _p, _p, _p, _p, _p]),
+    "d3f_unet_bn_on_stage": (_i, [_p, _i]),
     "d3f_conv_layer_plan": (_i, [_i, _desc, _i, _cvp]),
     "d3f_unet_num_conv_layers": (_i, [_p]),
     "d3f_unet_conv_layer": (_i, [_p, _i, _desc, _cvp]),
diff --git a/denoising_diffusion_deep_fake_amd/csrc/batchnorm.hip b/denoising_diffusion_deep_fake_amd/csrc/batchnorm.hip
--- a/denoising_diffusion_deep_fake_amd/csrc/batchnorm.hip
+++ b/denoising_diffusion_deep_fake_amd/csrc/batchnorm.hip
@@ -712,7 +712,7 @@
   const long min_rows = std::max(16L, 4L * (256 / std::max(1, std::min(256, L.C / (L.dtype == D3F_F32 ? 4 : 8)))));
   L.reduce_blocks = (int)std::clamp((L.rows + min_rows - 1) / min_rows, 1L, 1024L);
   L.bwd_rows = L.fused_rows > 0 ? L.fused_rows : L.reduce_blocks;
-  L.fwd_fused = L.apply && fused_ok(L.fwd_rows);
+  L.fwd_fused = L.apply && !L.on_stage && fused_ok(L.fwd_rows);
   L.bwd_fused = fused_ok(L.bwd_rows);
   L.rows_per_block = L.fwd_fused || L.bwd_fused ? rows_per_block_for(L.rows, L.C / BNF_SC, L.dtype, L.plan_nets) : 0;
   L.stat_floats = (size_t)L.fwd_rows * L.Cpad * 2;
@@ -761,7 +761,7 @@
     return bn_finalize_apply_launch(L, b, stream, ns);
   }
   if (int rc = bn_layer_finalize(L, b, count, stream, ns)) return rc;
-  return L.apply ? bn_layer_apply(L, b, stream, ns) : 0;
+  return (L.apply && !L.on_stage) ? bn_layer_apply(L, b, stream, ns) : 0;
 }
 
 int bn_layer_backward(const BnLayer& L, const BnBufs& b, const BnSync* sync, hipStream_t stream, const NetSplit* ns) {
diff --git a/denoising_diffusion_deep_fake_amd/csrc/c_api.hip b/denoising_diffusion_deep_fake_amd/csrc/c_api.hip
--- a/denoising_diffusion_deep_fake_amd/csrc/c_api.hip
+++ b/denoising_diffusion_deep_fake_amd/csrc/c_api.hip
@@ -540,6 +540,50 @@
                             (hipStream_t)stream);
 }
 
+static int plan_source_bn(ConvLayer& L, int dtype, const d3f_conv_desc* d, int what, bool head) {
+  L.head = head;
+  return plan(L, dtype, d, what);
+}
+int d3f_conv_source_bn_applies(int dtype, const d3f_conv_desc* d, int head) {
+  ConvLayer L;
+  if (d == nullptr || plan_source_bn(L, dtype, d, PLAN_FWD | PLAN_WGRAD, head != 0) != 0) return 0;
+  return (conv_patch_stages_bn(L.fwd, L.dtype) && wgrad_patch_stages_bn(L.wl, L.sdtype) && dtype == D3F_F32) ? 1 : 0;
+}
+int d3f_conv_forward_source_bn(int dtype, const d3f_conv_desc* d, const void* src_y, const float* src_coef,
+                               const void* w_fwd, void* out, float* stats, const float* bias, void* stream) {
+  ConvLayer L;
+  if (int rc = plan_source_bn(L, dtype, d, PLAN_FWD, bias != nullptr)) return rc;
+  if (d->B == 0) return 0;
+  D3F_CHECK(src_y && w_fwd && out && d->C1 == 0, "conv_forward_source_bn: null argument, or a second source");
+  D3F_CHECK(reinterpret_cast<uintptr_t>(src_coef) % 16 == 0 && (d->C0 % 4) == 0,
+            "conv_forward_source_bn: the coefficient block is read as 16-byte vectors");
+  ConvFwdBufs b;
+  b.src0 = src_y; b.w = w_fwd; b.out = out; b.stats = stats; b.bias = bias;
+  if (src_coef != nullptr) {
+    b.src_scale = bn_coef(src_coef, d->C0, BN_SCALE);
+    b.src_shift = bn_coef(src_coef, d->C0, BN_SHIFT);
+  }
+  return conv_layer_forward(L, b, false, (hipStream_t)stream);
+}
+int d3f_conv_backward_weight_source_bn(int dtype, const d3f_conv_desc* d, const void* dy, const void* src_y,
+                                       const float* src_coef, void* workspace, float* dw, void* stream) {
+  ConvLayer L;
+  if (int rc = plan(L, dtype, d, PLAN_WGRAD)) return rc;
+  D3F_CHECK(d->B > 0 && dy && src_y && src_coef && workspace && dw && d->C1 == 0,
+            "conv_backward_weight_source_bn: empty batch, null argument, or a second source");
+  D3F_CHECK(reinterpret_cast<uintptr_t>(src_coef) % 16 == 0 && (d->C0 % 4) == 0,
+            "conv_backward_weight_source_bn: the coefficient block is read as 16-byte vectors");
+  return wgrad_layer_launch(L.wl, dy, src_y, nullptr, reinterpret_cast<float*>(workspace), dw, d->Cout, d->CinReal, dtype,
+                            (hipStream_t)stream, bn_coef(src_coef, d->C0, BN_SCALE), bn_coef(src_coef, d->C0, BN_SHIFT));
+}
+int d3f_unet_bn_on_stage(d3f_unet_t h, int i) {
+  D3F_CHECK(h && i >= 0 && i < (int)h->e.bns.size(), "bn_on_stage: index %d", i);
+  int k = -1;
+  for (const Unit& u : h->e.units)
+    if (u.bn && ++k == i) return u.norm.on_stage ? 1 : 0;
+  return set_error(-1, "bn_on_stage: index %d", i);
+}
+
 static void conv_launch_out(const ConvParams& p, int dtype, d3f_conv_launch_plan* o) {
   const bool igemm = p.patch == 0, smallc = igemm && conv_igemm_small_c(p, dtype);
   o->planned = 1;
diff --git a/denoising_diffusion_deep_fake_amd/csrc/common.h b/denoising_diffusion_deep_fake_amd/csrc/common.h
--- a/denoising_diffusion_deep_fake_amd/csrc/common.h
+++ b/denoising_diffusion_deep_fake_amd/csrc/common.h
@@ -198,6 +198,8 @@
   int nets, plan_nets;
   long net_ws, net_out0, net_scale;
   int tile_bm, tile_bn;
+  const float* src_scale;
+  const float* src_shift;
 };
 __device__ __forceinline__ ConvParams conv_params_of_net(const ConvParams& pin, int net) {
   ConvParams p = pin;
@@ -207,6 +209,7 @@
     net_shift(p.stats, p.net_ws); net_shift(p.scale, p.net_scale); net_shift(p.shift, p.net_ws);
     net_shift(p.res, p.net_ws); net_shift(p.partial, p.net_ws);
     net_shift(p.bn_y, p.net_ws); net_shift(p.bn_coef, p.net_ws); net_shift(p.bn_partial, p.net_ws); net_shift(p.bn_a, p.net_ws);
+    net_shift(p.src_scale, p.net_ws); net_shift(p.src_shift, p.net_ws);
   }
   return p;
 }
@@ -229,6 +232,7 @@
 void conv_pres_plan(ConvParams& p);
 int conv_pres_launch(const ConvParams& p, hipStream_t stream);
 bool conv_patch_applies(const ConvParams& p, int dtype);
+bool conv_patch_stages_bn(const ConvParams& p, int dtype);
 bool conv_stem_applies(const ConvParams& p, int dtype);
 bool conv_stem_bf16_applies(const ConvParams& p, int dtype);
 void conv_patch_plan(ConvParams& p, int dtype);
@@ -259,11 +263,14 @@
   int step_img, step_row, step_col;
   int nets, plan_nets;
   long net_ws;
+  const float* src_scale;
+  const float* src_shift;
 };
 __device__ __forceinline__ WgradParams wgrad_params_of_net(const WgradParams& pin, int net) {
   WgradParams p = pin;
   if (net != 0) {
     net_shift(p.dy, p.net_ws); net_shift(p.src0, p.net_ws); net_shift(p.src1, p.net_ws); net_shift(p.partial, p.net_ws);
+    net_shift(p.src_scale, p.net_ws); net_shift(p.src_shift, p.net_ws);
   }
   return p;
 }
@@ -297,10 +304,13 @@
 int wgrad_layer_plan(WgradLayer& L, const WgradParams& base, int dtype);
 size_t wgrad_layer_partial_floats(const WgradLayer& L);
 int wgrad_layer_launch(const WgradLayer& L, const void* dy, const void* src0, const void* src1, float* partial,
-                       float* dw, int CoutReal, int CinReal, int dtype, hipStream_t stream);
+                       float* dw, int CoutReal, int CinReal, int dtype, hipStream_t stream,
+                       const float* src_scale = nullptr, const float* src_shift = nullptr);
 int wgrad_layer_launch_deferred(const WgradLayer& L, const void* dy, const void* src0, const void* src1, float* partial,
                                 float* dw, int CoutReal, int CinReal, int dtype, WgradReduceBatch& tb,
-                                hipStream_t stream, const NetSplit* ns = nullptr);
+                                hipStream_t stream, const NetSplit* ns = nullptr, const float* src_scale = nullptr,
+                                const float* src_shift = nullptr);
+bool wgrad_patch_stages_bn(const WgradLayer& L, int dtype);
 
 struct ConvLayer {
   int B = 0, Hv = 0, Wv = 0;
@@ -341,6 +351,8 @@
   const void* res = nullptr;
   int relu = 0;
   float* slabs = nullptr;
+  const float* src_scale = nullptr;
+  const float* src_shift = nullptr;
 };
 int conv_layer_forward(const ConvLayer& L, const ConvFwdBufs& b, bool wino, hipStream_t s, const NetSplit* ns = nullptr);
 struct ConvDgradBufs {
diff --git a/denoising_diffusion_deep_fake_amd/csrc/conv_igemm.hip b/denoising_diffusion_deep_fake_amd/csrc/conv_igemm.hip
--- a/denoising_diffusion_deep_fake_amd/csrc/conv_igemm.hip
+++ b/denoising_diffusion_deep_fake_amd/csrc/conv_igemm.hip
@@ -1446,6 +1446,9 @@
     D3F_CHECK(m0 == q.div_howo_mul && s0 == q.div_howo_shr && m1 == q.div_wo_mul && s1 == q.div_wo_shr,
               "conv: output extent changed after the plan (%d x %d)", q.Ho, q.Wo);
   }
+  D3F_CHECK((q.src_scale == nullptr && q.src_shift == nullptr) || conv_patch_stages_bn(q, dtype),
+            "conv: this launch's kernel cannot apply a source BatchNorm while staging (patch %d, C0 %d, mode %d)", q.patch,
+            q.C0, q.mode);
   const int prof_cls = q.mode == CONV_DGRAD ? PROF_CONV_DGRAD : PROF_CONV_FWD;
   const bool prof = prof_enabled(prof_cls);
   if (prof) prof_begin(prof_cls, q.flops, stream);
diff --git a/denoising_diffusion_deep_fake_amd/csrc/conv_patch.hip b/denoising_diffusion_deep_fake_amd/csrc/conv_patch.hip
--- a/denoising_diffusion_deep_fake_amd/csrc/conv_patch.hip
+++ b/denoising_diffusion_deep_fake_amd/csrc/conv_patch.hip
@@ -9,6 +9,10 @@
 static bool patch_conv_off() {
   static const bool off = getenv("D3F_NO_PATCH_CONV") != nullptr;
   return off;
+}
+
+bool conv_patch_stages_bn(const ConvParams& p, int dtype) {
+  return dtype == D3F_F32 && p.patch == 1 && p.C0 == 16 && (p.mode == CONV_RAW_STATS || p.mode == CONV_HEAD_NCHW);
 }
 
 bool conv_patch_applies(const ConvParams& p, int dtype) {
@@ -28,7 +32,7 @@
          (p.Wo % CP_PW) == 0 && p.Kpad >= 9 * p.C0;
 }
 
-template <typename T, int CIN, int BN, bool UP = false, int CSRC = CIN, bool SUM2 = false>
+template <typename T, int CIN, int BN, bool UP = false, int CSRC = CIN, bool SUM2 = false, bool XF = false>
 __global__ __launch_bounds__(256) void conv_patch_kernel(const ConvParams pin) {
   const ConvParams p = conv_params_of_net(pin, (int)blockIdx.z);
   chain_priority();
@@ -37,6 +41,7 @@
   static_assert(!UP || (W64 && BN == 16), "up-sampled source: bf16 x 32 channels -> 16 filters");
   static_assert(CSRC == CIN || (BF && CIN == 16 && CSRC == 8 && !UP), "half-filled pixels: bf16, 8 of 16 channels");
   static_assert(!SUM2 || (BF && CIN == 16 && CSRC == 16 && BN == 32 && !UP), "2x2-summed data gradient: bf16 x 16 -> 32");
+  static_assert(!XF || (!BF && CIN == 16 && CSRC == 16 && BN == 16 && !UP && !SUM2), "source transform: fp32 x 16 -> 16");
   static_assert(((CIN == 16 || (CIN == 4 && !BF)) && (BN == 16 || SUM2)) || (W64 && (BN == 32 || UP)),
                 "16 channels (forward / data gradient of decoder block 4, head forward), fp32 x 4 (data gradient of the "
                 "head) or bf16 x 32 -> 32 (decoder block 3 conv2)");
@@ -66,6 +71,7 @@
   const __amdgpu_buffer_rsrc_t rs = make_rsrc(p.src0, p.src0_bytes);
   const __amdgpu_buffer_rsrc_t rw = make_rsrc(p.w, p.w_bytes);
   uint4 pv[NLP], wv[NLW];
+  unsigned inside = 0;
 #pragma unroll
   for (int i = 0; i < NLP; ++i) {
     const int id = tid + 256 * i;
@@ -75,6 +81,13 @@
     const int Hs = UP ? p.H0s : p.Hv, Ws = UP ? p.W0s : p.Wv;
     const bool ok = id < NPV && (unsigned)gy < (unsigned)Hs && (unsigned)gx < (unsigned)Ws;
     pv[i] = buf_load16(rs, ok ? (unsigned)(((b * Hs + gy) * Ws + gx) * CSRC + cv * VEC) * (unsigned)sizeof(T) : BUF_OOB);
+    if constexpr (XF) inside |= (ok ? 1u : 0u) << i;
+  }
+  float4 xsc = make_float4(0.f, 0.f, 0.f, 0.f), xsf = xsc;
+  if constexpr (XF) {
+    static_assert(256 % CV == 0, "one channel vector per thread");
+    xsc = *reinterpret_cast<const float4*>(p.src_scale + (tid % CV) * VEC);
+    xsf = *reinterpret_cast<const float4*>(p.src_shift + (tid % CV) * VEC);
   }
 #pragma unroll
   for (int i = 0; i < NLW; ++i) {
@@ -95,6 +108,12 @@
           *reinterpret_cast<uint2*>(&P[pix * CS + 4]) = make_uint2(0u, 0u);
           *reinterpret_cast<uint2*>(&P[pix * CS + 6]) = make_uint2(0u, 0u);
         }
+      } else if constexpr (XF) {
+        float4 v = make_float4(__uint_as_float(pv[i].x), __uint_as_float(pv[i].y), __uint_as_float(pv[i].z), __uint_as_float(pv[i].w));
+        v.x = v.x * xsc.x + xsf.x; v.y = v.y * xsc.y + xsf.y; v.z = v.z * xsc.z + xsf.z; v.w = v.w * xsc.w + xsf.w;
+        v.x = fmaxf(v.x, 0.f); v.y = fmaxf(v.y, 0.f); v.z = fmaxf(v.z, 0.f); v.w = fmaxf(v.w, 0.f);
+        if (!((inside >> i) & 1u)) v = make_float4(0.f, 0.f, 0.f, 0.f);
+        *reinterpret_cast<float4*>(&P[pix * CS + cv * 4]) = v;
       } else {
         *reinterpret_cast<uint4*>(&P[pix * CS + cv * 4]) = pv[i];
       }
@@ -774,12 +793,18 @@
                 p.tiles_n == (p.patch == 4 ? cdiv(p.Cout, 32) : 1) &&
                 (p.shift0 == 0) == (p.patch != 5),
             "conv: patch params were not planned");
+  D3F_CHECK((p.src_scale == nullptr) == (p.src_shift == nullptr) &&
+                (p.src_scale == nullptr || (p.patch == 1 && p.C0 == 16 && (p.mode == CONV_RAW_STATS || p.mode == CONV_HEAD_NCHW))),
+            "conv: only the fp32 16-channel patch forward applies a source BatchNorm while staging (patch %d, C0 %d, mode %d)",
+            p.patch, p.C0, p.mode);
   const dim3 g1((unsigned)p.tiles_m, 1, (unsigned)nets_of(p.nets)), g2((unsigned)p.tiles_m, (unsigned)p.tiles_n, (unsigned)nets_of(p.nets));
   if (p.patch == 7) hipLaunchKernelGGL((conv_patch_kernel<bf16_t, 16, 32, false, 16, true>), g1, dim3(256), 0, stream, p);
   else if (p.patch == 6) hipLaunchKernelGGL((conv_patch_kernel<bf16_t, 16, 16, false, 8>), g1, dim3(256), 0, stream, p);
   else if (p.patch == 5) hipLaunchKernelGGL((conv_patch_kernel<bf16_t, 32, 16, true>), g1, dim3(256), 0, stream, p);
   else if (p.patch == 4) hipLaunchKernelGGL((conv_patch_kernel<bf16_t, 32, 32>), g2, dim3(256), 0, stream, p);
   else if (p.patch == 3) hipLaunchKernelGGL((conv_patch_kernel<bf16_t, 16, 16>), g1, dim3(256), 0, stream, p);
+  else if (p.C0 == 16 && p.src_scale != nullptr)
+    hipLaunchKernelGGL((conv_patch_kernel<float, 16, 16, false, 16, false, true>), g1, dim3(256), 0, stream, p);
   else if (p.C0 == 16) hipLaunchKernelGGL((conv_patch_kernel<float, 16, 16>), g1, dim3(256), 0, stream, p);
   else hipLaunchKernelGGL((conv_patch_kernel<float, 4, 16>), g1, dim3(256), 0, stream, p);
   D3F_HIP(hipGetLastError());
diff --git a/denoising_diffusion_deep_fake_amd/csrc/conv_plan.hip b/denoising_diffusion_deep_fake_amd/csrc/conv_plan.hip
--- a/denoising_diffusion_deep_fake_amd/csrc/conv_plan.hip
+++ b/denoising_diffusion_deep_fake_amd/csrc/conv_plan.hip
@@ -135,6 +135,9 @@
 int conv_layer_forward(const ConvLayer& L, const ConvFwdBufs& b, bool wino, hipStream_t s, const NetSplit* ns) {
   ConvParams p = L.fwd;
   p.src0 = b.src0; p.src1 = b.src1; p.w = b.w; p.out0 = b.out;
+  p.src_scale = b.src_scale; p.src_shift = b.src_shift;
+  D3F_CHECK(b.src_scale == nullptr || (!wino && b.scale == nullptr),
+            "conv forward: a source BatchNorm is applied while staging by the train-mode patch kernel only");
   net_conv(p, ns);
   if (L.head) {
     p.mode = CONV_HEAD_NCHW;
diff --git a/denoising_diffusion_deep_fake_amd/csrc/conv_wgrad.hip b/denoising_diffusion_deep_fake_amd/csrc/conv_wgrad.hip
--- a/denoising_diffusion_deep_fake_amd/csrc/conv_wgrad.hip
+++ b/denoising_diffusion_deep_fake_amd/csrc/conv_wgrad.hip
@@ -536,6 +536,8 @@
     if (prof) prof_end(stream);
     return rc;
   }
+  D3F_CHECK(p.src_scale == nullptr && p.src_shift == nullptr,
+            "wgrad: the tap-parallel kernel cannot apply a source BatchNorm while staging");
   const int t = pick_wtile(p);
   D3F_CHECK(p.tiles_co == cdiv(p.Cout, t) && p.splits >= 1 && p.slab_taps >= 1 && p.Mi >= 1, "wgrad: params were not planned");
   D3F_CHECK(!p.cls || t == 64, "wgrad: class form needs the 64x64 tile");
@@ -610,6 +612,11 @@
   return 0;
 }
 
+bool wgrad_patch_stages_bn(const WgradLayer& L, int dtype) {
+  const WgradParams& w = L.part[0];
+  return dtype == D3F_F32 && L.nparts == 1 && w.part == WG_WHOLE && w.patch == 2 && w.C1 == 0 && w.shift0 == 0;
+}
+
 size_t wgrad_layer_partial_floats(const WgradLayer& L) {
   size_t n = 0;
   for (int i = 0; i < L.nparts; ++i) n += (wgrad_partial_floats(L.part[i]) + 63) / 64 * 64;
@@ -618,7 +625,9 @@
 
 int wgrad_layer_launch_deferred(const WgradLayer& L, const void* dy, const void* src0, const void* src1, float* partial,
                                 float* dw, int CoutReal, int CinReal, int dtype, WgradReduceBatch& tb,
-                                hipStream_t stream, const NetSplit* ns) {
+                                hipStream_t stream, const NetSplit* ns, const float* src_scale, const float* src_shift) {
+  D3F_CHECK((src_scale == nullptr && src_shift == nullptr) || wgrad_patch_stages_bn(L, dtype),
+            "wgrad: this layer's kernel cannot apply a source BatchNorm while staging");
   if (ns != nullptr && ns->nets > 1) {
     tb.nets = ns->nets;
     tb.net_ws = ns->ws;
@@ -629,6 +638,7 @@
     w.dy = dy; w.src0 = src0; w.src1 = src1; w.partial = partial;
     w.nets = ns != nullptr ? ns->nets : 1;
     w.net_ws = ns != nullptr ? ns->ws : 0;
+    w.src_scale = src_scale; w.src_shift = src_shift;
     if (int rc = wgrad_launch(w, dtype, stream)) return rc;
     const int c_off = w.ci_base;
     const int creal = std::max(0, std::min(w.slab_cin, CinReal - c_off));
@@ -641,9 +651,12 @@
 }
 
 int wgrad_layer_launch(const WgradLayer& L, const void* dy, const void* src0, const void* src1, float* partial,
-                       float* dw, int CoutReal, int CinReal, int dtype, hipStream_t stream) {
+                       float* dw, int CoutReal, int CinReal, int dtype, hipStream_t stream, const float* src_scale,
+                       const float* src_shift) {
   WgradReduceBatch tb;
-  if (int rc = wgrad_layer_launch_deferred(L, dy, src0, src1, partial, dw, CoutReal, CinReal, dtype, tb, stream)) return rc;
+  if (int rc = wgrad_layer_launch_deferred(L, dy, src0, src1, partial, dw, CoutReal, CinReal, dtype, tb, stream, nullptr,
+                                           src_scale, src_shift))
+    return rc;
   return wgrad_reduce_batch_launch(tb, stream);
 }
 
diff --git a/denoising_diffusion_deep_fake_amd/csrc/conv_wgrad_patch.hip b/denoising_diffusion_deep_fake_amd/csrc/conv_wgrad_patch.hip
--- a/denoising_diffusion_deep_fake_amd/csrc/conv_wgrad_patch.hip
+++ b/denoising_diffusion_deep_fake_amd/csrc/conv_wgrad_patch.hip
@@ -27,11 +27,13 @@
   *reinterpret_cast<uint4*>(dst + 4) = make_uint4(v.z << 16, v.z & 0xffff0000u, v.w << 16, v.w & 0xffff0000u);
 }
 
-template <typename T, int MT, int CI_T, int KS, int S, int TW, int CR = CI_T>
+template <typename T, int MT, int CI_T, int KS, int S, int TW, int CR = CI_T, bool SRC_BN = false>
 __global__ __launch_bounds__(256) void conv_wgrad_patch_kernel(const WgradParams pin) {
   const WgradParams p = wgrad_params_of_net(pin, (int)blockIdx.z);
   constexpr int VE = Elem<T>::VE;
   constexpr int CO_T = MT;
+  static_assert(!SRC_BN || (sizeof(T) == 4 && MT == 16 && CI_T == 16 && KS == 3 && S == 1 && CR == CI_T),
+                "source transform: the fp32 16-channel 3x3 form");
   constexpr bool HALFV = CI_T < VE;
   static_assert(!HALFV || (CI_T == 4 && VE == 8), "half vectors: 4 of 8 bf16 channels");
   constexpr int PH = (PT_TH - 1) * S + KS, PW = (TW - 1) * S + KS;
@@ -90,10 +92,18 @@
 
   constexpr int NVX = (PH * PW * VX + 255) / 256, NVY = (PT_TH * TW * VY + 255) / 256;
   uint4 rxv[NVX], ryv[NVY];
+  unsigned inside = 0;
+  float4 xsc = make_float4(0.f, 0.f, 0.f, 0.f), xsf = xsc;
+  if constexpr (SRC_BN) {
+    static_assert(256 % VX == 0, "one channel vector per thread");
+    xsc = *reinterpret_cast<const float4*>(p.src_scale + cl0 + (tid % VX) * VE);
+    xsf = *reinterpret_cast<const float4*>(p.src_shift + cl0 + (tid % VX) * VE);
+  }
   auto issue_loads = [&](int t) {
     const int b = t / (tiles_y * tiles_x);
     const int tr = t - b * tiles_y * tiles_x;
     const int oy0 = (tr / tiles_x) * PT_TH, ox0 = (tr % tiles_x) * TW;
+    unsigned in_img = 0;
 #pragma unroll
     for (int i = 0; i < NVX; ++i) {
       const int v = tid + i * 256;
@@ -103,7 +113,9 @@
       const bool ok = v < PH * PW * VX && (unsigned)iy < (unsigned)p.Hv && (unsigned)ix < (unsigned)p.Wv;
       const int gp = (b * Hs + (iy >> sh)) * Ws + (ix >> sh);
       rxv[i] = buf_load16(rx, ok ? (unsigned)(gp * Cs + cl0 + cv * VE) * (unsigned)sizeof(T) : BUF_OOB);
-    }
+      if constexpr (SRC_BN) in_img |= (ok ? 1u : 0u) << i;
+    }
+    if constexpr (SRC_BN) inside = in_img;
 #pragma unroll
     for (int i = 0; i < NVY; ++i) {
       const int v = tid + i * 256;
@@ -121,11 +133,19 @@
       const int v = tid + i * 256;
       const int pix = v / VX, cv = v - pix * VX;
       if (v < PH * PW * VX) {
-        if constexpr (HALFV)
+        if constexpr (HALFV) {
           *reinterpret_cast<uint4*>(&Xs[pix * LXS]) =
               make_uint4(rxv[i].x << 16, rxv[i].x & 0xffff0000u, rxv[i].y << 16, rxv[i].y & 0xffff0000u);
-        else
+        } else if constexpr (SRC_BN) {
+          float4 a = make_float4(__uint_as_float(rxv[i].x), __uint_as_float(rxv[i].y), __uint_as_float(rxv[i].z),
+                                 __uint_as_float(rxv[i].w));
+          a.x = a.x * xsc.x + xsf.x; a.y = a.y * xsc.y + xsf.y; a.z = a.z * xsc.z + xsf.z; a.w = a.w * xsc.w + xsf.w;
+          a.x = fmaxf(a.x, 0.f); a.y = fmaxf(a.y, 0.f); a.z = fmaxf(a.z, 0.f); a.w = fmaxf(a.w, 0.f);
+          if (!((inside >> i) & 1u)) a = make_float4(0.f, 0.f, 0.f, 0.f);
+          *reinterpret_cast<float4*>(&Xs[pix * LXS + cv * VE]) = a;
+        } else {
           patch_store_f32<T>(&Xs[pix * LXS + cv * VE], rxv[i]);
+        }
       }
     }
 #pragma unroll
@@ -498,7 +518,15 @@
   const dim3 block(256);
   switch (variant) {
     case 1: hipLaunchKernelGGL((conv_wgrad_patch_kernel<T, 16, 32, 3, 1, 16>), grid, block, 0, stream, p); break;
-    case 2: hipLaunchKernelGGL((conv_wgrad_patch_kernel<T, 16, 16, 3, 1, 16>), grid, block, 0, stream, p); break;
+    case 2:
+      if constexpr (sizeof(T) == 4) {
+        if (p.src_scale != nullptr) {
+          hipLaunchKernelGGL((conv_wgrad_patch_kernel<T, 16, 16, 3, 1, 16, 16, true>), grid, block, 0, stream, p);
+          break;
+        }
+      }
+      hipLaunchKernelGGL((conv_wgrad_patch_kernel<T, 16, 16, 3, 1, 16>), grid, block, 0, stream, p);
+      break;
     case 3: hipLaunchKernelGGL((conv_wgrad_patch_kernel<T, 32, 32, 3, 1, 16>), grid, block, 0, stream, p); break;
     default: return set_error(-1, "wgrad patch: bad variant %d", variant);
   }
@@ -510,6 +538,10 @@
   wgrad_patch_grid(p, variant, &gx, &gy);
   D3F_CHECK(p.splits == gx, "wgrad patch: params were not planned (splits %d vs %d)", p.splits, gx);
   const dim3 grid((unsigned)gx, (unsigned)gy, (unsigned)nets_of(p.nets)), block(256);
+  D3F_CHECK((p.src_scale == nullptr) == (p.src_shift == nullptr) &&
+                (p.src_scale == nullptr || (variant == 2 && dtype == D3F_F32 && !p.cls && p.C1 == 0 && p.shift0 == 0)),
+            "wgrad patch: only the fp32 16-channel form (variant 2) applies a source BatchNorm while staging (variant %d)",
+            variant);
   if (p.cls) {
     D3F_CHECK((variant == 1 || variant == 3) && p.slab_cin == p.C0 && (p.C0 % 32) == 0 && (p.Ho % 2) == 0 && (p.Wo % 2) == 0,
               "wgrad patch: class form needs variant 1 or 3 and whole 32-channel slices of source 0");
diff --git a/denoising_diffusion_deep_fake_amd/csrc/engine.h b/denoising_diffusion_deep_fake_amd/csrc/engine.h
--- a/denoising_diffusion_deep_fake_amd/csrc/engine.h
+++ b/denoising_diffusion_deep_fake_amd/csrc/engine.h
@@ -33,6 +33,7 @@
   bool bn = true, bias = false;
   BnLayer norm;
   int res_tensor = -1, res_unit = -1;
+  int stage_bn = -1;
   long w_off = -1, bias_off = -1, g_off = -1, b_off = -1, rm_off = -1, rv_off = -1;
   size_t wf_off = 0, wd_off = 0;
   size_t coef_off = 0;
@@ -133,7 +134,7 @@
   int esize() const { return dtype == D3F_F32 ? 4 : 2; }
   int wsize() const { return cdtype == D3F_F32X3 ? 6 : esize(); }
   int ve() const { return dtype == D3F_F32 ? 4 : 8; }
-  const TensorD* find_export(const char* name) const;
+  bool find_export(const char* name, TensorD* t, const Unit** unit, std::string* kind) const;
   int new_tensor(int H_, int W_, int C_);
   int new_grad(int tensor_id);
   size_t alloc(size_t bytes);
@@ -217,6 +218,7 @@
   long pair_stride() const { return 2 * pair_fake_off(); }
   size_t head_nchw_off = 0;
   mutable bool head_z_live_ = false;
+  mutable bool staged_a_unwritten_ = false;
   size_t ws_top = 0;
   int t_x = -1, t_pool = -1, head = -1, conv1 = -1;
   size_t pool_idx_off = 0, stats_off = 0, bnpart_off = 0, dz_off = 0, dfull_off = 0,
diff --git a/denoising_diffusion_deep_fake_amd/csrc/engine.hip b/denoising_diffusion_deep_fake_amd/csrc/engine.hip
--- a/denoising_diffusion_deep_fake_amd/csrc/engine.hip
+++ b/denoising_diffusion_deep_fake_amd/csrc/engine.hip
@@ -364,6 +364,26 @@
     u.norm.mask = !op.mask ? BN_MASK_NONE : u.norm.res == BN_RES_NONE ? BN_MASK_FROM_Y : BN_MASK_FROM_A;
     u.norm.fused_rows = op.fused_rows;
   }
+  static const bool no_on_stage = getenv("D3F_NO_BN_ON_STAGE") != nullptr;
+  for (int pi = 0; pi < (int)units.size() && !no_on_stage; ++pi) {
+    Unit& u = units[pi];
+    if (!u.bn || u.a < 0 || !u.norm.apply || !u.norm.relu || u.norm.res != BN_RES_NONE || u.norm.mask != BN_MASK_FROM_Y ||
+        dtype != D3F_F32 || cdtype != D3F_F32 || u.a == units[conv1].a)
+      continue;
+    int consumers = 0;
+    bool ok = true;
+    for (const Unit& c : units) {
+      if (c.in1 == u.a || c.res_tensor == u.a) ok = false;
+      if (c.in0 != u.a) continue;
+      ++consumers;
+      ok = ok && c.in1 < 0 && !c.up0 && !c.upfold && c.C0 == u.Cout && conv_patch_stages_bn(c.fwd, c.dtype) &&
+           wgrad_patch_stages_bn(c.wl, c.sdtype);
+    }
+    if (!ok || consumers == 0) continue;
+    u.norm.on_stage = true;
+    for (Unit& c : units)
+      if (c.in0 == u.a) c.stage_bn = pi;
+  }
   for (Unit& u : units) {
     if (!u.bn) continue;
     bn_layer_plan(u.norm);
@@ -533,6 +553,7 @@
   auto coef = [&](const Unit& u) { return reinterpret_cast<float*>(ws + u.coef_off); };
   D3F_CHECK(ns == nullptr || (training && bn_sync() == nullptr), "unet: the pair engine runs train-mode passes with "
             "per-GPU BatchNorm statistics");
+  staged_a_unwritten_ = training != 0;
   if (!training) {
     BnEvalTable t;
     t.n = 0;
@@ -570,6 +591,12 @@
     b.src1 = u.in1 >= 0 ? T(u.in1) : nullptr;
     b.w = ws + (u.wino ? u.wu_off : u.upfold ? u.wfc_off : u.wf_off);
     b.slabs = reinterpret_cast<float*>(ws + splitk_off);
+    if (training && u.stage_bn >= 0) {
+      const Unit& pu = units[u.stage_bn];
+      b.src0 = T(pu.y);
+      b.src_scale = bn_coef(coef(pu), pu.Cout, BN_SCALE);
+      b.src_shift = bn_coef(coef(pu), pu.Cout, BN_SHIFT);
+    }
     if (!u.bn) {
       b.bias = params_ + u.bias_off;
       if (head_act_ == HEAD_ACT_IDENTITY || !apply_act) {
@@ -888,6 +915,7 @@
     g_step_ws_ = ws_;
   }
   D3F_HIP(hipGraphLaunch(g_step_, s));
+  staged_a_unwritten_ = true;
   return 0;
 }
 
@@ -932,6 +960,7 @@
   D3F_HIP(hipEventRecord(ev_gin_, s));
   D3F_HIP(hipStreamWaitEvent(gstream_, ev_gin_, 0));
   D3F_HIP(hipGraphLaunch(slot.exec, gstream_));
+  staged_a_unwritten_ = false;
   D3F_HIP(hipEventRecord(ev_gout_, gstream_));
   D3F_HIP(hipStreamWaitEvent(s, ev_gout_, 0));
   return 0;
@@ -1025,9 +1054,12 @@
     for (int ui : pending) {
       const Unit& u = units[ui];
       WgradReduceBatch red;
-      if (int rc = wgrad_layer_launch_deferred(u.wl, ws + u.dy_off, T(u.in0), u.in1 >= 0 ? T(u.in1) : nullptr,
+      const Unit* pu = u.stage_bn >= 0 ? &units[u.stage_bn] : nullptr;
+      if (int rc = wgrad_layer_launch_deferred(u.wl, ws + u.dy_off, pu ? T(pu->y) : T(u.in0), u.in1 >= 0 ? T(u.in1) : nullptr,
                                                reinterpret_cast<float*>(ws + u.wslab_off), grads + u.w_off, u.Cout,
-                                               u.CinReal, cdtype, red, ws_stream, ns))
+                                               u.CinReal, cdtype, red, ws_stream, ns,
+                                               pu ? bn_coef(coef(*pu), pu->Cout, BN_SCALE) : nullptr,
+                                               pu ? bn_coef(coef(*pu), pu->Cout, BN_SHIFT) : nullptr))
         return rc;
       if (!skip_r)
         if (int rc = wgrad_reduce_batch_launch(red, ws_stream)) return rc;
@@ -1125,33 +1157,52 @@
   return 0;
 }
 
-const TensorD* UnetEngine::find_export(const char* name) const {
+bool UnetEngine::find_export(const char* name, TensorD* t, const Unit** unit, std::string* kind_out) const {
   const std::string n(name);
   const size_t colon = n.rfind(':');
-  if (colon == std::string::npos) return nullptr;
+  if (colon == std::string::npos) return false;
   const std::string un = n.substr(0, colon), kind = n.substr(colon + 1);
-  if (kind != "y" && kind != "a" && kind != "da") return nullptr;
+  if (kind != "y" && kind != "a" && kind != "da" && kind != "dy") return false;
   for (const Unit& u : units) {
     if (u.conv_name != un) continue;
+    *unit = &u;
+    *kind_out = kind;
+    if (kind == "dy") {
+      t->off = u.dy_off; t->H = u.Ho; t->W = u.Wo; t->C = u.CoutD;
+      return true;
+    }
     const int tid = kind == "y" ? u.y : u.a;
-    if (tid < 0) return nullptr;
-    if (kind == "da") return grad_of[tid] >= 0 ? &gtensors[grad_of[tid]] : nullptr;
-    return &tensors[tid];
-  }
-  return nullptr;
+    if (tid < 0) return false;
+    if (kind == "da" && grad_of[tid] < 0) return false;
+    *t = kind == "da" ? gtensors[grad_of[tid]] : tensors[tid];
+    return true;
+  }
+  return false;
 }
 
 int UnetEngine::export_tensor(const char* name, const void* ws_, float* out_nchw, hipStream_t s) const {
-  const TensorD* t = find_export(name);
-  D3F_CHECK(t != nullptr, "export: no tensor named '%s' (expected '<conv name>:y|a|da')", name);
-  return nhwc_to_nchw_launch(dtype, reinterpret_cast<const char*>(ws_) + t->off, out_nchw, B, t->C, t->H, t->W, t->C, s);
+  TensorD t;
+  const Unit* u = nullptr;
+  std::string kind;
+  D3F_CHECK(find_export(name, &t, &u, &kind), "export: no tensor named '%s' (expected '<conv name>:y|a|da|dy')", name);
+  if (kind == "a" && u->norm.on_stage && staged_a_unwritten_) {
+    char* ws = const_cast<char*>(reinterpret_cast<const char*>(ws_));
+    BnBufs n;
+    n.coef = reinterpret_cast<float*>(ws + u->coef_off);
+    n.y = ws + tensors[u->y].off;
+    n.a = ws + tensors[u->a].off;
+    if (int rc = bn_layer_apply(u->norm, n, s)) return rc;
+  }
+  return nhwc_to_nchw_launch(dtype, reinterpret_cast<const char*>(ws_) + t.off, out_nchw, B, t.C, t.H, t.W, t.C, s);
 }
 
 int UnetEngine::export_shape(const char* name, int32_t dims[3]) const {
-  const TensorD* t = find_export(name);
-  D3F_CHECK(t != nullptr, "export: no tensor named '%s' (expected '<conv name>:y|a|da')", name);
-  dims[0] = t->C; dims[1] = t->H; dims[2] = t->W;
-  return 0;
-}
-
-}
+  TensorD t;
+  const Unit* u = nullptr;
+  std::string kind;
+  D3F_CHECK(find_export(name, &t, &u, &kind), "export: no tensor named '%s' (expected '<conv name>:y|a|da|dy')", name);
+  dims[0] = t.C; dims[1] = t.H; dims[2] = t.W;
+  return 0;
+}
+
+}
diff --git a/denoising_diffusion_deep_fake_amd/csrc/pointwise.h b/denoising_diffusion_deep_fake_amd/csrc/pointwise.h
--- a/denoising_diffusion_deep_fake_amd/csrc/pointwise.h
+++ b/denoising_diffusion_deep_fake_amd/csrc/pointwise.h
@@ -38,6 +38,7 @@
   int fwd_rows = 0;
   int fused_rows = 0;
   bool allow_fused = false;
+  bool on_stage = false;
   bool fwd_fused = false, bwd_fused = false;
   int reduce_blocks = 0;
   int bwd_rows = 0;
diff --git a/include/d3f_hip.h b/include/d3f_hip.h
--- a/include/d3f_hip.h
+++ b/include/d3f_hip.h
@@ -146,6 +146,13 @@
 int d3f_conv_backward_weight(int dtype, const d3f_conv_desc* d, const void* dy, const void* src0,
                              const void* src1, void* workspace, float* dw, void* stream);
 
+int d3f_conv_source_bn_applies(int dtype, const d3f_conv_desc* d, int head);
+int d3f_conv_forward_source_bn(int dtype, const d3f_conv_desc* d, const void* src_y, const float* src_coef,
+                               const void* w_fwd, void* out, float* stats, const float* bias, void* stream);
+int d3f_conv_backward_weight_source_bn(int dtype, const d3f_conv_desc* d, const void* dy, const void* src_y,
+                                       const float* src_coef, void* workspace, float* dw, void* stream);
+int d3f_unet_bn_on_stage(d3f_unet_t h, int i);
+
 typedef struct d3f_conv_launch_plan {
   int32_t planned;
   int32_t patch;
```

Result: no change. 2084 images/sec (-0.0%).
